# auduno/headtrackr

Hardware: AMD Instinct MI355X
Metric: frames/sec full-cascade detect at 320x240 (higher is better)
Workload: dtype u8; 1 GPU; C2: 256 x 320x240 RGBA frames per GPU, full BBF cascade detect (interval 5) incl. grouping + best face per frame on the host; frames_per_gpu=256, frames_total=256, width=320, height=240, batches_in_flight=3, parallelism=1 GPU

## Files before the change

### headtrackr_amd/csrc/ht_context.hip

```cpp
#include <sched.h>
#include <algorithm>
#include <cmath>
#include <cstddef>
#include <cstdlib>
#include <cstring>
#include <new>

#include "ht_internal.h"
#include "ht_hostpost.h"
#include "ht_geometry_plan.h"
#include "ht_cascade_plan.h"

static thread_local std::string g_create_err;

#include <dlfcn.h>
namespace {
struct Roctx {
    int (*push)(const char *) = nullptr;
    int (*pop)() = nullptr;
    Roctx() {
        void *h = dlopen("libroctx64.so", RTLD_NOW | RTLD_GLOBAL);
        if (!h) h = dlopen("libroctx64.so.4", RTLD_NOW | RTLD_GLOBAL);
        if (h) {
            push = reinterpret_cast<int (*)(const char *)>(dlsym(h, "roctxRangePushA"));
            pop = reinterpret_cast<int (*)()>(dlsym(h, "roctxRangePop"));
            if (!push || !pop) push = nullptr, pop = nullptr;
        }
    }
};
Roctx &roctx() {
    static Roctx r;
    return r;
}
}
HtRange::HtRange(const char *name) : on(roctx().push != nullptr) {
    if (on) roctx().push(name);
}
HtRange::~HtRange() {
    if (on) roctx().pop();
}

#include <atomic>
#include <mutex>
static std::mutex g_live_mu;
static std::vector<ht_ctx *> g_live;
struct HtOrphan {
    void *p;
    size_t bytes;
    int device;
    bool orphan;
};
static std::vector<HtOrphan> g_orphans;
static std::atomic<int> g_orphan_count{0};

static bool bound_by_live_context(const ht_ctx *except, int device, const void *p, size_t bytes) {
    const uint8_t *pb = static_cast<const uint8_t *>(p);
    for (const ht_ctx *o : g_live)
        if (o != except && o->device == device && o->d_frames && o->d_frames >= pb && o->d_frames < pb + bytes) return true;
    return false;
}

static void sweep_orphans(ht_ctx *c) {
    if (g_orphan_count.load(std::memory_order_relaxed) == 0) return;
    std::vector<HtOrphan> release;
    {
        std::lock_guard<std::mutex> lk(g_live_mu);
        for (size_t i = 0; i < g_orphans.size();) {
            if (!bound_by_live_context(nullptr, g_orphans[i].device, g_orphans[i].p, g_orphans[i].bytes)) {
                release.push_back(g_orphans[i]);
                g_orphans.erase(g_orphans.begin() + (long)i);
            } else {
                i++;
            }
        }
        g_orphan_count.store((int)g_orphans.size(), std::memory_order_relaxed);
    }
    for (auto &a : release) {
        (void)hipSetDevice(a.device);
        (void)hipDeviceSynchronize();
        (void)hipFree(a.p);
    }
    if (!release.empty() && c) (void)hipSetDevice(c->device);
}

static inline HtPostCfg post_cfg(const ht_ctx *c) { return HtPostCfg{c->interval, c->cascade.cw, c->cascade.ch}; }

static int ht_host_workers(const ht_ctx *c, int frames, uint32_t hits) {
    if (c->host_threads == 0) return 0;
    if (c->host_threads > 0) return c->host_threads;
    if (frames < 32 || hits < 256) return 0;
    static const int share = [] {
        cpu_set_t set;
        CPU_ZERO(&set);
        int cpus = sched_getaffinity(0, sizeof(set), &set) == 0 ? CPU_COUNT(&set) : (int)std::thread::hardware_concurrency();
        int ngpu = 1;
        if (hipGetDeviceCount(&ngpu) != hipSuccess || ngpu < 1) ngpu = 1;
        return std::max(0, std::min(7, cpus / (2 * ngpu) - 1));
    }();
    return share;
}


ht_status ht_fail(ht_ctx *ctx, ht_status st, const std::string &msg) {
    if (ctx)
        ctx->err = msg;
    else
        g_create_err = msg;
    return st;
}

HtProfScope::HtProfScope(ht_ctx *c, const char *name, hipStream_t on) : ctx(c), stream(on ? on : c->stream) {
    if (!ctx->profiling) return;
    for (size_t i = 0; i < ctx->timers.size(); i++)
        if (ctx->timers[i].name == name) idx = (int)i;
    if (idx < 0) {
        ctx->timers.emplace_back();
        ctx->timers.back().name = name;
        idx = (int)ctx->timers.size() - 1;
    }
    if (hipEventCreate(&a) != hipSuccess || hipEventCreate(&b) != hipSuccess) {
        idx = -1;
        return;
    }
    (void)hipEventRecord(a, stream);
}
HtProfScope::~HtProfScope() {
    if (idx < 0) return;
    (void)hipEventRecord(b, stream);
    ctx->timers[idx].pending.emplace_back(a, b);
    ctx->timers[idx].launches++;
}

extern "C" int32_t ht_abi_version(void) { return HT_ABI_VERSION; }

extern "C" const char *ht_last_error(const ht_ctx *ctx) { return ctx ? ctx->err.c_str() : g_create_err.c_str(); }

static bool apply_options(ht_ctx *c, const std::string &opts, std::string &why) {
    size_t pos = 0;
    while (pos < opts.size()) {
        size_t end = opts.find(',', pos);
        if (end == std::string::npos) end = opts.size();
        std::string kv = opts.substr(pos, end - pos);
        pos = end + 1;
        while (!kv.empty() && (kv.front() == ' ')) kv.erase(kv.begin());
        while (!kv.empty() && (kv.back() == ' ')) kv.pop_back();
        if (kv.empty()) continue;
        const size_t eq = kv.find('=');
        const std::string key = kv.substr(0, eq), val = eq == std::string::npos ? "1" : kv.substr(eq + 1);
        char *endp = nullptr;
        const long long v = std::strtoll(val.c_str(), &endp, 10);
        if (val.empty() || (endp && *endp)) {
            why = "option '" + key + "': value is not an integer";
            return false;
        }
        const int iv = (int)std::max<long long>(std::min<long long>(v, 1ll << 30), -(1ll << 30));
        if (key == "rs_rpt") { if (iv >= 1 && iv <= HT_RS_MAX_PASSES) c->rs_rpt = iv; }
        else if (key == "rs_tailtable") c->tail_table = iv < 0 ? 0 : (iv > 2 ? 2 : (int)iv), c->tail_table_forced = true;
        else if (key == "rs_tailcap") c->rs_tailcap = (uint64_t)std::max<long long>(v, 0), c->rs_tailcap_forced = true;
        else if (key == "rs_notail") c->rs_notail = iv != 0;
        else if (key == "rs_nofast") c->rs_nofast = iv != 0;
        else if (key == "rs_nosort") c->rs_nosort = iv != 0;
        else if (key == "rs_bands") c->rs_bands = iv != 0;
        else if (key == "rs_gennames") c->rs_gennames = iv != 0;
        else if (key == "rs_minwg") c->rs_min_wgs = std::max(1, iv);
        else if (key == "rs_k") c->dbg_rs_k = iv;
        else if (key == "rs_group") { if (iv >= 1 && iv <= 64) c->rs_group = iv, c->rs_group_forced = true; }
        else if (key == "early_scan") c->early_scan = iv != 0;
        else if (key == "force_exact") c->dbg_force_exact = iv;
        else if (key == "deep_bias") c->deep_bias = (uint32_t)std::max(0, iv);
        else if (key == "deep_v") c->dbg_deep_v = iv;
        else if (key == "cs_flags") c->cs_flags = iv != 0;
        else if (key == "cs_sync_ring") c->cs_sync_ring = iv != 0;
        else if (key == "cs_pairs_force") c->cs_pairs_force = iv != 0;
        else if (key == "cs_pairs_cluster") c->cs_pairs_cluster = iv != 0;
        else if (key == "fp_sparse") c->fp_sparse = iv != 0;
        else if (key == "deep_grid") c->deep_grid = std::max(1, iv);
        else if (key == "split") c->opt_split = std::max(1, iv);
        else if (key == "cs_fused_min") c->cs_fused_min_streams = std::max(1, iv);
        else if (key == "cs_fused_nt") c->cs_fused_nt = iv;
        else if (key == "cs_keep_hist") c->cs_keep_hist = iv != 0;
        else if (key == "cs_seq_fused") c->cs_seq_fused = iv != 0;
        else if (key == "cs_cluster") c->cs_cluster = iv != 0;
        else if (key == "cs_cluster_min_px") c->cs_cluster_min_px = (uint32_t)std::max(0, iv);
        else if (key == "cs_region") c->cs_region_cap = std::min(40960, std::max(0, iv));
        else if (key == "cs_barrier_budget") c->cs_barrier_budget = std::max(1ll, v);
        else if (key == "graph_max_frames") c->graph_max_frames = std::max(0, iv);
        else if (key == "host_threads") c->host_threads = std::min(64, std::max(0, iv));
        else if (key == "force_rccl") c->force_rccl = iv != 0;
        else if (key == "group_cap") c->grp_cap_opt = std::max(1, iv);
#ifdef HT_DEBUG_KNOBS
        else if (key == "stop_stage") c->dbg_stop_stage = iv;
        else if (key == "cs_iters") c->dbg_cs_iters = std::min(10, std::max(0, iv));
        else if (key == "rs_maxgen") c->rs_maxgen = iv;
#endif
        else {
            why = "unknown option '" + key + "'";
            return false;
        }
    }
    return true;
}

template <typename T>
static ht_status upload_table(ht_ctx *c, T *&dst, const std::vector<T> &src) {
    if (src.empty()) return HT_OK;
    HT_HIP(c, hipMalloc(&dst, src.size() * sizeof(T)));
    HT_HIP(c, hipMemcpy(dst, src.data(), src.size() * sizeof(T), hipMemcpyHostToDevice));
    return HT_OK;
}

extern "C" ht_status ht_create(const ht_config *cfg, const void *cascade_blob, size_t cascade_len, ht_ctx **out) {
    if (!cfg || !out || (cfg->struct_size != sizeof(ht_config) && cfg->struct_size != offsetof(ht_config, options)))
        return ht_fail(nullptr, HT_ERR_INVALID, "ht_create: bad config");
    *out = nullptr;
    if (cfg->interval < 1 || cfg->interval > 12) return ht_fail(nullptr, HT_ERR_INVALID, "ht_create: interval must be 1..12");
    int ndev = 0;
    if (hipGetDeviceCount(&ndev) != hipSuccess || ndev <= 0)
        return ht_fail(nullptr, HT_ERR_NO_DEVICE, "ht_create: no HIP device visible (this library has no CPU fallback)");
    if (cfg->device < 0 || cfg->device >= ndev) return ht_fail(nullptr, HT_ERR_INVALID, "ht_create: device ordinal out of range");
    hipDeviceProp_t prop;
    if (hipGetDeviceProperties(&prop, cfg->device) != hipSuccess) return ht_fail(nullptr, HT_ERR_HIP, "hipGetDeviceProperties failed");
    if (std::strncmp(prop.gcnArchName, "gfx950", 6) != 0)
        return ht_fail(nullptr, HT_ERR_NO_DEVICE, std::string("ht_create: device is ") + prop.gcnArchName + ", this build is gfx950-only");
    ht_ctx *c = new (std::nothrow) ht_ctx();
    if (!c) return ht_fail(nullptr, HT_ERR_NOMEM, "ht_create: out of host memory");
    c->device = cfg->device;
    c->num_cus = prop.multiProcessorCount > 0 ? prop.multiProcessorCount : 256;
    c->interval = cfg->interval;
    c->next = cfg->interval + 1;
    if (cfg->hit_capacity) c->hit_capacity = cfg->hit_capacity;
    c->queue_capacity_cfg = cfg->queue_capacity;
    std::string why;
    if (!ht_plan_cascade((const uint8_t *)cascade_blob, cascade_len, &c->cascade, &why)) {
        delete c;
        return ht_fail(nullptr, HT_ERR_INVALID, "ht_create: " + why);
    }
    ht_status st = HT_OK;
    auto bail = [&](ht_status s) {
        g_create_err = c->err;
        ht_destroy(c);
        return s;
    };
    if (hipSetDevice(c->device) != hipSuccess) {
        c->err = "hipSetDevice failed";
        return bail(HT_ERR_HIP);
    }
    if (cfg->stream) {
        c->stream = (hipStream_t)cfg->stream;
    } else {
        if (hipStreamCreateWithFlags(&c->stream, hipStreamNonBlocking) != hipSuccess) {
            c->err = "hipStreamCreate failed";
            return bail(HT_ERR_HIP);
        }
        c->own_stream = true;
    }
    {
        std::string opts = (cfg->struct_size >= offsetof(ht_config, options) + sizeof(const char *) && cfg->options) ? cfg->options : "";
#ifdef HT_DEBUG_KNOBS
        if (const char *e = std::getenv("HT_OPTIONS")) opts += std::string(opts.empty() ? "" : ",") + e;
#endif
        std::string why;
        if (!apply_options(c, opts, why)) {
            c->err = "ht_create: " + why;
            return bail(HT_ERR_INVALID);
        }
    }
    if (c->early_scan) {
        if (hipStreamCreateWithFlags(&c->aux_stream, hipStreamNonBlocking) != hipSuccess || hipEventCreateWithFlags(&c->ev_early_ready, hipEventDisableTiming) != hipSuccess ||
            hipEventCreateWithFlags(&c->ev_early_done, hipEventDisableTiming) != hipSuccess) {
            c->err = "hipStreamCreate (aux) failed";
            return bail(HT_ERR_HIP);
        }
    }
    c->builtin_cascade = ht_scan_is_builtin_cascade((const uint8_t *)cascade_blob, cascade_len) && c->interval >= 1;
    ht_plan_cascade_split(&c->cascade, c->builtin_cascade, c->opt_split);
    const HtCascadePlan &P = c->cascade;
    if ((st = upload_table(c, c->d_deep_feats, P.deep)) != HT_OK || (st = upload_table(c, c->d_stages, P.dev_stages)) != HT_OK ||
        (st = upload_table(c, c->d_tile_feats, P.tile)) != HT_OK || (st = upload_table(c, c->d_fp_feats, P.fp)) != HT_OK ||
        (st = upload_table(c, c->d_patch_feats, P.patch)) != HT_OK || (st = upload_table(c, c->d_packed_feats, P.packed)) != HT_OK)
        return bail(st);
    if (hipHostMalloc(reinterpret_cast<void **>(&c->h_pinned), sizeof(HtCounters) + (size_t)HT_PINNED_HITS * sizeof(ht_hit), hipHostMallocDefault) != hipSuccess ||
        hipMalloc(&c->d_stats, sizeof(unsigned long long) * 64 * HT_STAT_SHARDS) != hipSuccess ||
        hipMalloc(reinterpret_cast<void **>(&c->d_counters), sizeof(HtCounters) + (size_t)c->hit_capacity * sizeof(ht_hit)) != hipSuccess) {
        c->err = "hipMalloc(hits) failed";
        return bail(HT_ERR_NOMEM);
    }
    {
        std::lock_guard<std::mutex> lk(g_live_mu);
        g_live.push_back(c);
    }
    c->d_hits = reinterpret_cast<ht_hit *>(reinterpret_cast<uint8_t *>(c->d_counters) + sizeof(HtCounters));
    *out = c;
    return HT_OK;
}

static void destroy_graphs(ht_ctx *c);
static void free_geometry(ht_ctx *c) {
    destroy_graphs(c);
    if (c->d_levels) (void)hipFree(c->d_levels), c->d_levels = nullptr;
    if (c->d_arena) (void)hipFree(c->d_arena), c->d_arena = nullptr;
    if (c->d_scales) (void)hipFree(c->d_scales), c->d_scales = nullptr;
    if (c->d_queue) (void)hipFree(c->d_queue), c->d_queue = nullptr;
    for (auto p : c->d_gen_blocks)
        if (p) (void)hipFree(p);
    c->d_gen_blocks.clear();
    if (c->d_tile_recs) (void)hipFree(c->d_tile_recs), c->d_tile_recs = nullptr;
    if (c->d_tail_jobs) (void)hipFree(c->d_tail_jobs), c->d_tail_jobs = nullptr;
    if (c->d_tail_prefix) (void)hipFree(c->d_tail_prefix), c->d_tail_prefix = nullptr;
    if (c->d_tail_taps) (void)hipFree(c->d_tail_taps), c->d_tail_taps = nullptr;
    if (c->d_tail_taps_fast) (void)hipFree(c->d_tail_taps_fast), c->d_tail_taps_fast = nullptr;
    if (c->d_tail_tapref) (void)hipFree(c->d_tail_tapref), c->d_tail_tapref = nullptr;
    c->plan.tail_first_gen = 0;
    c->plan.gens.clear();
    c->plan.gen_blocks.clear();
    c->plan.scales.clear();
}

extern "C" void ht_destroy(ht_ctx *c) {
    if (!c) return;
    std::vector<HtOrphan> release;
    {
        std::lock_guard<std::mutex> lk(g_live_mu);
        g_live.erase(std::remove(g_live.begin(), g_live.end(), c), g_live.end());
        for (auto &a : c->user_allocs) {
            if (bound_by_live_context(c, c->device, a.first, a.second)) g_orphans.push_back(HtOrphan{a.first, a.second, c->device, true});
            else release.push_back(HtOrphan{a.first, a.second, c->device, false});
        }
        c->user_allocs.clear();
        for (size_t i = 0; i < g_orphans.size();) {
            if (!bound_by_live_context(nullptr, g_orphans[i].device, g_orphans[i].p, g_orphans[i].bytes)) {
                release.push_back(g_orphans[i]);
                g_orphans.erase(g_orphans.begin() + (long)i);
            } else {
                i++;
            }
        }
        g_orphan_count.store((int)g_orphans.size(), std::memory_order_relaxed);
    }
    (void)hipSetDevice(c->device);
    if (c->stream) (void)hipStreamSynchronize(c->stream);
    if (c->aux_stream) (void)hipStreamSynchronize(c->aux_stream), (void)hipStreamDestroy(c->aux_stream);
    if (c->ev_early_ready) (void)hipEventDestroy(c->ev_early_ready);
    if (c->ev_early_done) (void)hipEventDestroy(c->ev_early_done);
    free_geometry(c);
    if (c->d_tile_feats) (void)hipFree(c->d_tile_feats);
    if (c->d_deep_feats) (void)hipFree(c->d_deep_feats);
    if (c->d_patch_feats) (void)hipFree(c->d_patch_feats);
    if (c->d_packed_feats) (void)hipFree(c->d_packed_feats);
    if (c->d_fp_feats) (void)hipFree(c->d_fp_feats);
    if (c->d_stages) (void)hipFree(c->d_stages);
    if (c->d_frames_own) (void)hipFree(c->d_frames_own);
    if (c->d_frames_back) (void)hipFree(c->d_frames_back);
    if (c->ev_copy_done) (void)hipEventDestroy(c->ev_copy_done);
    if (c->ev_front_free) (void)hipEventDestroy(c->ev_front_free);
    if (c->copy_stream) (void)hipStreamDestroy(c->copy_stream);
    if (c->d_counters) (void)hipFree(c->d_counters);
    if (c->d_stats) (void)hipFree(c->d_stats);
    if (c->h_pinned) (void)hipHostFree(c->h_pinned);
    if (c->d_scratch) (void)hipFree(c->d_scratch);
    if (c->h_wb_pinned) (void)hipHostFree(c->h_wb_pinned);
    ht_camshift_free(c);
    ht_backproject_free(c);
    ht_ingest_free(c);
    ht_cs_pairs_free(c);
    ht_cs_best_free(c);
    ht_group_free(c);
    if (c->d_gather) (void)hipFree(c->d_gather);
    for (auto &a : release) {
        if (a.orphan) {
            (void)hipSetDevice(a.device);
            (void)hipDeviceSynchronize();
        }
        (void)hipFree(a.p);
    }
    (void)hipSetDevice(c->device);
    for (auto &t : c->timers)
        for (auto &p : t.pending) (void)hipEventDestroy(p.first), (void)hipEventDestroy(p.second);
    if (c->own_stream && c->stream) (void)hipStreamDestroy(c->stream);
    delete c;
}


static ht_status set_geometry_impl(ht_ctx *c, int32_t width, int32_t height, int32_t max_batch, const int32_t *level_dims, int n, int upto) {
    c->W = width;
    c->H = height;
    c->max_batch = max_batch;
    c->nlevels = n;
    c->upto = upto;

    HtPlanInputs in;
    in.interval = c->interval, in.next = c->next, in.cw = c->cascade.cw, in.ch = c->cascade.ch;
    in.rs_rpt = c->rs_rpt, in.rs_nofast = c->rs_nofast, in.rs_nosort = c->rs_nosort, in.rs_notail = c->rs_notail;
    in.rs_tailcap = c->rs_tailcap, in.rs_tailcap_forced = c->rs_tailcap_forced;
    in.tail_table = c->tail_table, in.tail_table_forced = c->tail_table_forced;
    in.early_scan = c->early_scan, in.aux_stream = c->aux_stream != nullptr;
    in.queue_capacity_cfg = c->queue_capacity_cfg;
    HtGeometryPlan &P = c->plan;
    std::string why;
    ht_status st = ht_plan_geometry(in, width, height, max_batch, level_dims, n, upto, &P, &why);
    if (st != HT_OK) return ht_fail(c, st, why);

    c->d_gen_blocks.assign(P.gens.size(), nullptr);
    for (size_t g = 1; g < P.gens.size(); g++)
        if ((st = upload_table(c, c->d_gen_blocks[g], P.gen_tiles[g])) != HT_OK) return st;
    HT_HIP(c, hipMalloc(&c->d_levels, sizeof(HtDevLevel) * HT_MAX_LEVELS));
    HT_HIP(c, hipMemcpy(c->d_levels, P.levels, sizeof(HtDevLevel) * n, hipMemcpyHostToDevice));
    if (hipMalloc(&c->d_arena, P.arena_stride * (uint64_t)max_batch) != hipSuccess)
        return ht_fail(c, HT_ERR_NOMEM, "ht_set_geometry: hipMalloc(pyramid arena) failed");
    HT_HIP(c, hipMemset(c->d_arena, 0, P.arena_stride * (uint64_t)max_batch));
    if ((st = upload_table(c, c->d_tail_jobs, P.tail_jobs)) != HT_OK || (st = upload_table(c, c->d_tail_prefix, P.tail_prefix)) != HT_OK ||
        (st = upload_table(c, c->d_tail_taps, P.tail_taps)) != HT_OK || (st = upload_table(c, c->d_tail_taps_fast, P.tail_taps_fast)) != HT_OK ||
        (st = upload_table(c, c->d_tail_tapref, P.tail_tapref)) != HT_OK || (st = upload_table(c, c->d_tile_recs, P.tile_recs)) != HT_OK ||
        (st = upload_table(c, c->d_scales, P.scales)) != HT_OK)
        return st;
    if (hipMalloc(&c->d_queue, (size_t)P.queue_capacity * sizeof(HtQueueEntry) + HT_DEEP_CTR_BYTES) != hipSuccess)
        return ht_fail(c, HT_ERR_NOMEM, "ht_set_geometry: hipMalloc(survivor queue) failed");
    return HT_OK;
}

extern "C" ht_status ht_set_geometry(ht_ctx *c, int32_t width, int32_t height, int32_t max_batch, const int32_t *level_dims,
                                     int32_t nlevels_in) {
    if (!c) return HT_ERR_INVALID;
    if (width <= 0 || height <= 0 || width > 16384 || height > 16384 || max_batch <= 0)
        return ht_fail(c, HT_ERR_INVALID, "ht_set_geometry: width/height must be 1..16384 and max_batch > 0");
    HT_HIP(c, hipSetDevice(c->device));
    const int upto = (int)std::floor(std::log((double)std::min(c->cascade.cw, c->cascade.ch)) / std::log(ht_scale_of(c->interval)));
    const int n = upto + c->next * 2;
    if (n > HT_MAX_LEVELS) return ht_fail(c, HT_ERR_INVALID, "ht_set_geometry: too many pyramid levels");
    if (level_dims && nlevels_in != n) return ht_fail(c, HT_ERR_INVALID, "ht_set_geometry: level_dims has the wrong number of levels");
    if (level_dims)
        for (int i = 0; i < n; i++) {
            const int lw = level_dims[2 * i], lh = level_dims[2 * i + 1];
            if (lw < 0 || lh < 0 || lw > width || lh > height || (i == 0 && (lw != width || lh != height)))
                return ht_fail(c, HT_ERR_INVALID, "ht_set_geometry: bad level_dims");
        }
    if (c->W == width && c->H == height && c->max_batch >= max_batch && c->nlevels == n && !level_dims) return HT_OK;
    HT_HIP(c, hipStreamSynchronize(c->stream));
    if (c->copy_stream) HT_HIP(c, hipStreamSynchronize(c->copy_stream));
    free_geometry(c);
    c->nframes = c->enq_nframes = 0;
    c->wb_collected_n = -1;
    c->back_n = 0;
    c->d_frames = nullptr;
    c->enqueued = false;
    const ht_status st = set_geometry_impl(c, width, height, max_batch, level_dims, n, upto);
    if (st != HT_OK) {
        (void)hipGetLastError();
        free_geometry(c);
        c->W = c->H = c->max_batch = c->nlevels = c->upto = 0;
    }
    return st;
}

extern "C" int32_t ht_num_levels(const ht_ctx *c) { return c ? c->nlevels : 0; }
extern "C" uint64_t ht_windows_per_frame(const ht_ctx *c) { return c ? c->plan.windows_per_frame : 0; }
extern "C" uint64_t ht_pyramid_bytes_per_frame(const ht_ctx *c) { return c ? c->plan.pyr_bytes : 0; }

extern "C" ht_status ht_plane(const ht_ctx *c, int32_t level, int32_t slot, ht_plane_info *out) {
    if (!c || !out || level < 0 || level >= c->nlevels || slot < 0 || slot > 3) return HT_ERR_INVALID;
    const HtDevLevel &L = c->plan.levels[level];
    out->width = L.w;
    out->height = L.h;
    out->stride = L.stride;
    out->present = L.off[slot] != 0xffffffffu;
    out->offset = out->present ? L.off[slot] : 0;
    return HT_OK;
}


extern "C" ht_status ht_upload_frames(ht_ctx *c, const uint8_t *host_rgba, int32_t n, size_t frame_stride) {
    if (!c) return HT_ERR_INVALID;
    HtRange range("ht_upload_frames");
    if (c->W == 0) return ht_fail(c, HT_ERR_STATE, "ht_upload_frames: call ht_set_geometry first");
    const size_t fbytes = (size_t)c->W * c->H * 4;
    if (!host_rgba || n <= 0 || n > c->max_batch || frame_stride < fbytes)
        return ht_fail(c, HT_ERR_INVALID, "ht_upload_frames: bad frame count or stride");
    HT_HIP(c, hipSetDevice(c->device));
    const size_t need = fbytes * (size_t)n;
    const ht_status st = ht_frames_own_reserve(c, need, "ht_upload_frames");
    if (st != HT_OK) return st;
    if (frame_stride == fbytes) {
        HT_HIP(c, hipMemcpyAsync(c->d_frames_own, host_rgba, need, hipMemcpyHostToDevice, c->stream));
    } else {
        HT_HIP(c, hipMemcpy2DAsync(c->d_frames_own, fbytes, host_rgba, frame_stride, fbytes, (size_t)n, hipMemcpyHostToDevice, c->stream));
    }
    ht_frames_bind_own(c, n);
    return HT_OK;
}

ht_status ht_frames_own_reserve(ht_ctx *c, size_t need, const char *fn) {
    if (c->d_frames_own_bytes >= need) return HT_OK;
    HT_HIP(c, hipStreamSynchronize(c->stream));
    if (c->d_frames == c->d_frames_own) c->d_frames = nullptr, c->nframes = 0;
    if (c->d_frames_own) (void)hipFree(c->d_frames_own);
    c->d_frames_own = nullptr;
    c->d_frames_own_bytes = 0;
    if (hipMalloc(&c->d_frames_own, need) != hipSuccess) return (void)hipGetLastError(), ht_fail(c, HT_ERR_NOMEM, std::string(fn) + ": hipMalloc failed");
    c->d_frames_own_bytes = need;
    return HT_OK;
}
void ht_frames_bind_own(ht_ctx *c, int n) {
    c->d_frames = c->d_frames_own;
    c->frame_stride = (size_t)c->W * c->H * 4;
    c->nframes = n;
    sweep_orphans(c);
}

extern "C" ht_status ht_upload_frames_async(ht_ctx *c, const uint8_t *host_rgba, int32_t n, size_t frame_stride) {
    if (!c) return HT_ERR_INVALID;
    if (c->W == 0) return ht_fail(c, HT_ERR_STATE, "ht_upload_frames_async: call ht_set_geometry first");
    const size_t fbytes = (size_t)c->W * c->H * 4;
    if (!host_rgba || n <= 0 || n > c->max_batch || frame_stride < fbytes)
        return ht_fail(c, HT_ERR_INVALID, "ht_upload_frames_async: bad frame count or stride");
    HT_HIP(c, hipSetDevice(c->device));
    if (!c->copy_stream) {
        HT_HIP(c, hipStreamCreateWithFlags(&c->copy_stream, hipStreamNonBlocking));
        HT_HIP(c, hipEventCreateWithFlags(&c->ev_copy_done, hipEventDisableTiming));
        HT_HIP(c, hipEventCreateWithFlags(&c->ev_front_free, hipEventDisableTiming));
    }
    const size_t need = fbytes * (size_t)n;
    if (c->d_frames_back_bytes < need) {
        HT_HIP(c, hipStreamSynchronize(c->copy_stream));
        if (c->d_frames_back) (void)hipFree(c->d_frames_back);
        c->d_frames_back = nullptr;
        c->d_frames_back_bytes = 0;
        if (hipMalloc(&c->d_frames_back, need) != hipSuccess) return ht_fail(c, HT_ERR_NOMEM, "ht_upload_frames_async: hipMalloc failed");
        c->d_frames_back_bytes = need;
    }
    HT_HIP(c, hipStreamWaitEvent(c->copy_stream, c->ev_front_free, 0));
    if (frame_stride == fbytes) {
        HT_HIP(c, hipMemcpyAsync(c->d_frames_back, host_rgba, need, hipMemcpyHostToDevice, c->copy_stream));
    } else {
        HT_HIP(c, hipMemcpy2DAsync(c->d_frames_back, fbytes, host_rgba, frame_stride, fbytes, (size_t)n, hipMemcpyHostToDevice, c->copy_stream));
    }
    HT_HIP(c, hipEventRecord(c->ev_copy_done, c->copy_stream));
    c->back_n = n;
    return HT_OK;
}

extern "C" ht_status ht_swap_frames(ht_ctx *c) {
    if (!c) return HT_ERR_INVALID;
    if (c->back_n <= 0) return ht_fail(c, HT_ERR_STATE, "ht_swap_frames: no ht_upload_frames_async pending");
    HT_HIP(c, hipSetDevice(c->device));
    HT_HIP(c, hipEventRecord(c->ev_front_free, c->stream));
    HT_HIP(c, hipStreamWaitEvent(c->stream, c->ev_copy_done, 0));
    std::swap(c->d_frames_own, c->d_frames_back);
    std::swap(c->d_frames_own_bytes, c->d_frames_back_bytes);
    c->d_frames = c->d_frames_own;
    c->frame_stride = (size_t)c->W * c->H * 4;
    c->nframes = c->back_n;
    c->back_n = 0;
    sweep_orphans(c);
    return HT_OK;
}

extern "C" ht_status ht_bind_frames_device(ht_ctx *c, const void *dev_rgba, int32_t n, size_t frame_stride) {
    if (!c) return HT_ERR_INVALID;
    if (c->W == 0) return ht_fail(c, HT_ERR_STATE, "ht_bind_frames_device: call ht_set_geometry first");
    if (!dev_rgba || n <= 0 || n > c->max_batch || frame_stride < (size_t)c->W * c->H * 4 || (frame_stride & 3) ||
        ((uintptr_t)dev_rgba & 3))
        return ht_fail(c, HT_ERR_INVALID, "ht_bind_frames_device: bad pointer, frame count or stride (4-byte alignment required)");
    c->d_frames = (const uint8_t *)dev_rgba;
    c->frame_stride = frame_stride;
    c->nframes = n;
    sweep_orphans(c);
    return HT_OK;
}

extern "C" int32_t ht_frames_bound(const ht_ctx *c) { return c ? c->nframes : 0; }
extern "C" int32_t ht_frames_enqueued(const ht_ctx *c) { return (c && c->enqueued) ? c->enq_nframes : 0; }

extern "C" ht_status ht_host_alloc(size_t bytes, void **out) {
    if (!out || bytes == 0) return HT_ERR_INVALID;
    *out = nullptr;
    if (hipHostMalloc(out, bytes, hipHostMallocDefault) != hipSuccess) {
        (void)hipGetLastError();
        return ht_fail(nullptr, HT_ERR_NOMEM, "ht_host_alloc: hipHostMalloc failed");
    }
    return HT_OK;
}
extern "C" void ht_host_free(void *p) {
    if (p) (void)hipHostFree(p);
}
extern "C" ht_status ht_device_alloc(ht_ctx *c, size_t bytes, void **out) {
    if (!c || !out || bytes == 0) return HT_ERR_INVALID;
    *out = nullptr;
    HT_HIP(c, hipSetDevice(c->device));
    if (hipMalloc(out, bytes) != hipSuccess) {
        (void)hipGetLastError();
        return ht_fail(c, HT_ERR_NOMEM, "ht_device_alloc: hipMalloc failed");
    }
    c->user_allocs.emplace_back(*out, bytes);
    return HT_OK;
}
extern "C" ht_status ht_device_free(ht_ctx *c, void *p) {
    if (!c) return HT_ERR_INVALID;
    if (!p) return HT_OK;
    HT_HIP(c, hipSetDevice(c->device));
    HT_HIP(c, hipStreamSynchronize(c->stream));
    auto it = std::find_if(c->user_allocs.begin(), c->user_allocs.end(), [p](const std::pair<void *, size_t> &a) { return a.first == p; });
    if (it == c->user_allocs.end()) return ht_fail(c, HT_ERR_INVALID, "ht_device_free: not a live ht_device_alloc buffer of this context");
    const uint8_t *pb = static_cast<const uint8_t *>(p);
    {
        std::lock_guard<std::mutex> lk(g_live_mu);
        if (bound_by_live_context(c, c->device, pb, it->second))
            return ht_fail(c, HT_ERR_STATE, "ht_device_free: another live context still has frames bound inside this buffer (rebind or destroy it first)");
    }
    if (c->d_frames && c->d_frames >= pb && c->d_frames < pb + it->second) {
        c->d_frames = nullptr, c->nframes = 0;
        destroy_graphs(c);
    }
    c->user_allocs.erase(it);
    HT_HIP(c, hipFree(p));
    sweep_orphans(c);
    return HT_OK;
}
extern "C" ht_status ht_device_upload(ht_ctx *c, void *dst_dev, const void *src_host, size_t bytes) {
    if (!c || !dst_dev || !src_host) return HT_ERR_INVALID;
    if (bytes == 0) return HT_OK;
    HT_HIP(c, hipSetDevice(c->device));
    HT_HIP(c, hipMemcpyAsync(dst_dev, src_host, bytes, hipMemcpyHostToDevice, c->stream));
    HT_HIP(c, hipStreamSynchronize(c->stream));
    return HT_OK;
}

extern "C" ht_status ht_device_download(ht_ctx *c, void *dst_host, const void *src_dev, size_t bytes) {
    if (!c || !dst_host || !src_dev) return HT_ERR_INVALID;
    if (bytes == 0) return HT_OK;
    HT_HIP(c, hipSetDevice(c->device));
    HT_HIP(c, hipMemcpyAsync(dst_host, src_dev, bytes, hipMemcpyDeviceToHost, c->stream));
    HT_HIP(c, hipStreamSynchronize(c->stream));
    return HT_OK;
}


static ht_status wb_scratch(ht_ctx *c) {
    const size_t region = sizeof(unsigned long long) * 4 * (size_t)std::max(c->max_batch, 1), need = 2 * region;
    if (c->d_scratch_bytes < need) {
        HT_HIP(c, hipStreamSynchronize(c->stream));
        destroy_graphs(c);
        if (c->d_scratch) (void)hipFree(c->d_scratch);
        c->d_scratch = nullptr;
        c->d_scratch_bytes = 0;
        if (hipMalloc(&c->d_scratch, need) != hipSuccess) return ht_fail(c, HT_ERR_NOMEM, "whitebalance scratch: hipMalloc failed");
        c->d_scratch_bytes = need;
    }
    if (c->h_wb_pinned_bytes < region) {
        HT_HIP(c, hipStreamSynchronize(c->stream));
        if (c->h_wb_pinned) (void)hipHostFree(c->h_wb_pinned);
        c->h_wb_pinned = nullptr;
        c->h_wb_pinned_bytes = 0;
        if (hipHostMalloc(reinterpret_cast<void **>(&c->h_wb_pinned), region, hipHostMallocDefault) != hipSuccess)
            return ht_fail(c, HT_ERR_NOMEM, "whitebalance staging: hipHostMalloc failed");
        c->h_wb_pinned_bytes = region;
    }
    return HT_OK;
}
static unsigned long long *wb_standalone_region(ht_ctx *c) {
    return reinterpret_cast<unsigned long long *>(c->d_scratch) + 4 * (size_t)std::max(c->max_batch, 1);
}

static ht_status detect_enqueue_body(ht_ctx *c, uint32_t flags) {
    HT_HIP(c, hipMemsetAsync(c->d_counters, 0, sizeof(HtCounters), c->stream));
    c->early_launched = false;
    if (flags & HT_SCAN_STATS) HT_HIP(c, hipMemsetAsync(c->d_stats, 0, sizeof(unsigned long long) * 64 * HT_STAT_SHARDS, c->stream));
    ht_status st;
    c->wb_fused = false;
    const bool wb = (flags & HT_DETECT_WHITEBALANCE) != 0;
    if (wb) {
        HT_HIP(c, hipMemsetAsync(c->d_scratch, 0, sizeof(unsigned long long) * 4 * (size_t)c->nframes, c->stream));
        c->wb_fused = (c->W & 3) == 0;
    }
    st = ht_launch_pyramid(c, flags);
    c->wb_fused = false;
    if (st != HT_OK) return st;
    if (wb && (c->W & 3) != 0 && (st = ht_launch_whitebalance(c, c->d_scratch, false)) != HT_OK) return st;
    return ht_launch_scan(c, flags);
}

static void destroy_graphs(ht_ctx *c) {
    for (auto &g : c->graphs) {
        if (g.exec) (void)hipGraphExecDestroy(g.exec);
        if (g.graph) (void)hipGraphDestroy(g.graph);
    }
    c->graphs.clear();
}

extern "C" uint64_t ht_graph_launches(const ht_ctx *c) { return c ? c->graph_launches : 0; }

extern "C" ht_status ht_detect_enqueue(ht_ctx *c, uint32_t flags) {
    if (!c) return HT_ERR_INVALID;
    HtRange range("ht_detect_enqueue");
    if (!c->d_frames || c->nframes <= 0) return ht_fail(c, HT_ERR_STATE, "ht_detect_enqueue: no frames bound");
    HT_HIP(c, hipSetDevice(c->device));
    ht_status st;
    if ((flags & HT_DETECT_WHITEBALANCE) && (st = wb_scratch(c)) != HT_OK) return st;
    const bool graph_ok = c->graph_max_frames > 0 && c->nframes <= c->graph_max_frames && c->own_stream && !c->profiling && !c->early_scan &&
                          !(flags & HT_SCAN_STATS);
    bool done = false;
    if (graph_ok) {
        HtDetectGraph *g = nullptr;
        for (auto &e : c->graphs)
            if (e.frames == c->d_frames && e.frame_stride == c->frame_stride && e.nframes == c->nframes && e.flags == flags) g = &e;
        if (!g) {
            if (c->graphs.size() >= 8) {
                HtDetectGraph &old = c->graphs.front();
                if (old.exec) (void)hipGraphExecDestroy(old.exec);
                if (old.graph) (void)hipGraphDestroy(old.graph);
                c->graphs.erase(c->graphs.begin());
            }
            c->graphs.emplace_back();
            g = &c->graphs.back();
            g->frames = c->d_frames, g->frame_stride = c->frame_stride, g->nframes = c->nframes, g->flags = flags;
        }
        if (!g->exec && g->seen == 1) {
            ht_capture_mark(c, true);
            if (hipStreamBeginCapture(c->stream, hipStreamCaptureModeThreadLocal) == hipSuccess) {
                st = detect_enqueue_body(c, flags);
                hipGraph_t graph = nullptr;
                const hipError_t e = hipStreamEndCapture(c->stream, &graph);
                ht_capture_mark(c, false);
                if (st == HT_OK && e == hipSuccess && graph && hipGraphInstantiate(&g->exec, graph, nullptr, nullptr, 0) == hipSuccess) {
                    g->graph = graph;
                } else {
                    if (graph) (void)hipGraphDestroy(graph);
                    g->exec = nullptr;
                    g->seen = 1 << 30;
                    (void)hipGetLastError();
                }
            } else {
                ht_capture_mark(c, false);
                (void)hipGetLastError();
                g->seen = 1 << 30;
            }
        }
        if (g->exec) {
            HT_HIP(c, hipGraphLaunch(g->exec, c->stream));
            c->graph_launches++;
            c->early_launched = false;
            done = true;
        } else if (g->seen < (1 << 30)) {
            g->seen++;
        }
    }
    if (!done && (st = detect_enqueue_body(c, flags)) != HT_OK) return st;
    c->stats_enqueued = (flags & HT_SCAN_STATS) != 0;
    c->wb_enqueued = (flags & HT_DETECT_WHITEBALANCE) != 0;
    c->enqueued = true;
    c->grp_enqueued = false;
    c->enq_nframes = c->nframes;
    return HT_OK;
}

ht_status ht_detect_mark_collected(ht_ctx *c, bool wb_snap) {
    c->enqueued = false;
    if (wb_snap) {
        c->h_wb_sums.assign(c->h_wb_pinned, c->h_wb_pinned + 4 * (size_t)c->enq_nframes);
        c->wb_collected_n = c->enq_nframes;
    } else {
        c->wb_collected_n = -1;
    }
    std::memset(c->h_stage_in, 0, sizeof(c->h_stage_in));
    if (c->stats_enqueued) {
        std::vector<unsigned long long> sh((size_t)64 * HT_STAT_SHARDS);
        HT_HIP(c, hipMemcpy(sh.data(), c->d_stats, sh.size() * sizeof(unsigned long long), hipMemcpyDeviceToHost));
        for (int r = 0; r < HT_STAT_SHARDS; r++)
            for (int j = 0; j < 64; j++) c->h_stage_in[j] += sh[(size_t)r * 64 + j];
    }
    return HT_OK;
}

static inline bool hit_less(const ht_hit &a, const ht_hit &b) {
    if (a.frame != b.frame) return a.frame < b.frame;
    if (a.scale != b.scale) return a.scale < b.scale;
    if (a.q != b.q) return a.q < b.q;
    if (a.y != b.y) return a.y < b.y;
    return a.x < b.x;
}

extern "C" ht_status ht_detect_collect(ht_ctx *c, ht_hit *hits, uint32_t cap, uint32_t *counts, uint32_t *total) {
    if (!c) return HT_ERR_INVALID;
    HtRange range("ht_detect_collect");
    if (!c->enqueued) return ht_fail(c, HT_ERR_STATE, "ht_detect_collect: nothing enqueued");
    HT_HIP(c, hipSetDevice(c->device));
    uint32_t spec = std::max<uint32_t>(256u, 64u * (uint32_t)std::max(c->enq_nframes, 1));
    if (c->spec_hint) spec = std::min(spec, std::max<uint32_t>(256u, c->spec_hint + c->spec_hint / 2 + 64u));
    spec = std::min<uint32_t>(spec, std::min<uint32_t>(HT_PINNED_HITS, c->hit_capacity));
    HT_HIP(c, hipMemcpyAsync(c->h_pinned, c->d_counters, sizeof(HtCounters) + (size_t)spec * sizeof(ht_hit), hipMemcpyDeviceToHost, c->stream));
    const bool wb_snap = c->wb_enqueued && c->h_wb_pinned;
    if (wb_snap)
        HT_HIP(c, hipMemcpyAsync(c->h_wb_pinned, c->d_scratch, sizeof(unsigned long long) * 4 * (size_t)c->enq_nframes, hipMemcpyDeviceToHost, c->stream));
    HT_HIP(c, hipStreamSynchronize(c->stream));
    std::memcpy(&c->h_counters, c->h_pinned, sizeof(HtCounters));
    c->grp_enqueued = false;
    const ht_status cst = ht_detect_mark_collected(c, wb_snap);
    if (cst != HT_OK) return cst;
    const uint32_t found = c->h_counters.nhits;
    c->spec_hint = found;
    if (total) *total = found;
    const uint32_t nfr = (uint32_t)c->enq_nframes;
    if (counts) std::memset(counts, 0, sizeof(uint32_t) * (size_t)nfr);
    if (found > c->hit_capacity)
        return ht_fail(c, HT_ERR_CAPACITY, "ht_detect_collect: more raw hits than ht_config.hit_capacity; results incomplete");
    std::vector<ht_hit> &tmp = c->h_raw_hits;
    tmp.resize(found);
    if (found) {
        const uint32_t have = std::min(found, spec);
        std::memcpy(tmp.data(), c->h_pinned + sizeof(HtCounters), (size_t)have * sizeof(ht_hit));
        if (found > have)
            HT_HIP(c, hipMemcpy(tmp.data() + have, c->d_hits + have, (size_t)(found - have) * sizeof(ht_hit), hipMemcpyDeviceToHost));
    }
    if (c->requeue_flags >= 0) {
        const uint32_t fl = (uint32_t)c->requeue_flags;
        c->requeue_flags = -1;
        ht_status rq = ht_detect_enqueue(c, fl);
        if (rq != HT_OK) return rq;
    }
    const uint32_t ncopy = std::min(found, cap);
    ht_hit *dst = hits;
    if (found && (!hits || cap < found)) {
        c->h_ordered_hits.resize(found);
        dst = c->h_ordered_hits.data();
    }
    bool bucketed = found > 0 && nfr > 0;
    if (bucketed) {
        bucketed = ht_post_bucket_by_frame(tmp.data(), found, nfr, dst, c->h_frame_start, counts);
        if (bucketed) {
            const uint32_t *se = c->h_frame_start.data();
            if (c->collect_best_follows) {
                c->h_sort_deferred = true;
            } else {
                auto sort_frames = [&](int f0, int f1) {
                    for (int f = f0; f < f1; f++) ht_post_sort_frame(dst, f ? se[f - 1] : 0u, se[f]);
                };
                const int nw = ht_host_workers(c, (int)nfr, found);
                if (nw > 0) HtPool::get().run((int)nfr, 16, nw, sort_frames);
                else sort_frames(0, (int)nfr);
            }
        }
    }
    if (found && !bucketed) {
        std::sort(tmp.begin(), tmp.end(), hit_less);
        if (counts) {
            std::memset(counts, 0, sizeof(uint32_t) * (size_t)nfr);
            for (uint32_t i = 0; i < found; i++)
                if (tmp[i].frame < nfr) counts[tmp[i].frame]++;
        }
        std::memcpy(dst, tmp.data(), (size_t)found * sizeof(ht_hit));
    }
    if (found && dst != hits && hits && ncopy) std::memcpy(hits, dst, (size_t)ncopy * sizeof(ht_hit));
    if (found > cap) return ht_fail(c, HT_ERR_CAPACITY, "ht_detect_collect: caller buffer too small for all hits");
    return HT_OK;
}

extern "C" ht_status ht_detect_batch(ht_ctx *c, const uint8_t *host_rgba, int32_t n, int32_t width, int32_t height, size_t frame_stride,
                                     uint32_t flags, ht_hit *hits, uint32_t cap, uint32_t *counts, uint32_t *total) {
    if (!c) return HT_ERR_INVALID;
    ht_status st;
    if (c->W != width || c->H != height || c->max_batch < n)
        if ((st = ht_set_geometry(c, width, height, n, nullptr, 0)) != HT_OK) return st;
    if ((st = ht_upload_frames(c, host_rgba, n, frame_stride)) != HT_OK) return st;
    if ((st = ht_detect_enqueue(c, flags)) != HT_OK) return st;
    return ht_detect_collect(c, hits, cap, counts, total);
}

extern "C" ht_status ht_pyramid_readback(ht_ctx *c, int32_t frame, int32_t level, int32_t slot, uint8_t *out, size_t cap) {
    if (!c || !out) return HT_ERR_INVALID;
    if (frame < 0 || frame >= c->max_batch || level < 0 || level >= c->nlevels || slot < 0 || slot > 3)
        return ht_fail(c, HT_ERR_INVALID, "ht_pyramid_readback: index out of range");
    const HtDevLevel &L = c->plan.levels[level];
    if (L.off[slot] == 0xffffffffu) return ht_fail(c, HT_ERR_INVALID, "ht_pyramid_readback: plane does not exist");
    if (cap < (size_t)L.w * L.h) return ht_fail(c, HT_ERR_CAPACITY, "ht_pyramid_readback: buffer too small");
    if (L.w == 0 || L.h == 0) return HT_OK;
    HT_HIP(c, hipSetDevice(c->device));
    HT_HIP(c, hipStreamSynchronize(c->stream));
    HT_HIP(c, hipMemcpy2D(out, L.w, c->d_arena + (uint64_t)frame * c->plan.arena_stride + L.off[slot], L.stride, L.w, L.h, hipMemcpyDeviceToHost));
    return HT_OK;
}

extern "C" ht_status ht_stage_counts(ht_ctx *c, uint64_t *counts, int32_t n) {
    if (!c || !counts || n < (int32_t)c->cascade.nstages + 1) return HT_ERR_INVALID;
    for (uint32_t j = 0; j <= c->cascade.nstages; j++) counts[j] = c->h_stage_in[j];
    for (int32_t j = (int32_t)c->cascade.nstages + 1; j < std::min<int32_t>(n, 64); j++) counts[j] = c->h_stage_in[j];
    return HT_OK;
}

extern "C" ht_status ht_grayscale_batch(ht_ctx *c, uint8_t *host_rgba, int32_t n, int32_t width, int32_t height, size_t frame_stride) {
    if (!c || !host_rgba || n <= 0 || width <= 0 || height <= 0 || frame_stride < (size_t)width * height * 4) return HT_ERR_INVALID;
    HT_HIP(c, hipSetDevice(c->device));
    const size_t fbytes = (size_t)width * height * 4;
    uint8_t *d = nullptr;
    if (hipMalloc(&d, fbytes * n) != hipSuccess) return ht_fail(c, HT_ERR_NOMEM, "ht_grayscale_batch: hipMalloc failed");
    ht_status st = HT_OK;
    hipError_t e = hipMemcpy2DAsync(d, fbytes, host_rgba, frame_stride, fbytes, n, hipMemcpyHostToDevice, c->stream);
    if (e == hipSuccess) {
        const int W0 = c->W, H0 = c->H;
        c->W = width, c->H = height;
        st = ht_launch_gray_inplace(c, d, n, fbytes);
        c->W = W0, c->H = H0;
    }
    if (e == hipSuccess && st == HT_OK) e = hipMemcpy2DAsync(host_rgba, frame_stride, d, fbytes, fbytes, n, hipMemcpyDeviceToHost, c->stream);
    if (e == hipSuccess) e = hipStreamSynchronize(c->stream);
    (void)hipFree(d);
    if (e != hipSuccess) return ht_fail(c, HT_ERR_HIP, std::string("ht_grayscale_batch: ") + hipGetErrorString(e));
    return st;
}

static void wb_values(const ht_ctx *c, const unsigned long long *sums, double *out, int32_t n) {
    const double imagesize = (double)c->W * (double)c->H;
    for (int i = 0; i < n; i++) {
        const double avgr = (double)sums[4 * i] / imagesize, avgg = (double)sums[4 * i + 1] / imagesize, avgb = (double)sums[4 * i + 2] / imagesize;
        out[i] = (avgr + avgg + avgb) / 3;
    }
}

extern "C" ht_status ht_whitebalance_batch(ht_ctx *c, double *out, int32_t n) {
    if (!c || !out) return HT_ERR_INVALID;
    if (!c->d_frames || n <= 0 || n > c->nframes) return ht_fail(c, HT_ERR_STATE, "ht_whitebalance_batch: no frames bound");
    HT_HIP(c, hipSetDevice(c->device));
    ht_status st = wb_scratch(c);
    if (st != HT_OK) return st;
    unsigned long long *d_sums = wb_standalone_region(c);
    if ((st = ht_launch_whitebalance(c, reinterpret_cast<double *>(d_sums), true)) != HT_OK) return st;
    std::vector<unsigned long long> sums((size_t)n * 4);
    HT_HIP(c, hipMemcpyAsync(sums.data(), d_sums, sizeof(unsigned long long) * 4 * (size_t)n, hipMemcpyDeviceToHost, c->stream));
    HT_HIP(c, hipStreamSynchronize(c->stream));
    wb_values(c, sums.data(), out, n);
    return HT_OK;
}

extern "C" ht_status ht_detect_whitebalance(ht_ctx *c, double *out, int32_t n) {
    if (!c || !out) return HT_ERR_INVALID;
    if (c->wb_collected_n < 0)
        return ht_fail(c, HT_ERR_STATE, "ht_detect_whitebalance: the batch collected last was not enqueued with HT_DETECT_WHITEBALANCE (call after ht_detect_collect)");
    if (n <= 0 || n > c->wb_collected_n) return ht_fail(c, HT_ERR_INVALID, "ht_detect_whitebalance: n exceeds the collected batch");
    wb_values(c, c->h_wb_sums.data(), out, n);
    return HT_OK;
}


extern "C" ht_status ht_hits_to_rects(const ht_ctx *c, const ht_hit *hits, uint32_t n, ht_rect *out) {
    if (!c || (n && (!hits || !out))) return HT_ERR_INVALID;
    const HtPostCfg cfg = post_cfg(c);
    double sx[HT_MAX_LEVELS];
    ht_post_level_scales(cfg, sx);
    return ht_post_hits_to_rects(cfg, sx, hits, n, out);
}

extern "C" ht_status ht_group_rects(const ht_rect *seq, uint32_t n, int32_t min_neighbors, ht_rect *out, uint32_t *nout) {
    return ht_post_group_rects(seq, n, min_neighbors, out, nout);
}

extern "C" ht_status ht_best_faces(const ht_ctx *c, const ht_hit *hits, const uint32_t *counts, int32_t nframes, int32_t min_neighbors,
                                   ht_rect *best) {
    if (!c || !counts || !best || nframes < 0) return HT_ERR_INVALID;
    const HtPostCfg cfg = post_cfg(c);
    double sx[HT_MAX_LEVELS];
    ht_post_level_scales(cfg, sx);
    size_t k = 0;
    for (int f = 0; f < nframes; f++) {
        const ht_status st = ht_post_best_face(cfg, sx, hits ? hits + k : nullptr, counts[f], min_neighbors, &best[f]);
        if (st != HT_OK) return st;
        k += counts[f];
    }
    return HT_OK;
}

extern "C" ht_status ht_detect_collect_best(ht_ctx *c, int32_t min_neighbors, ht_rect *best, uint32_t *total_hits) {
    if (!c || !best) return HT_ERR_INVALID;
    HtRange range("ht_detect_collect_best");
    if (!c->enqueued) return ht_fail(c, HT_ERR_STATE, "ht_detect_collect_best: nothing enqueued");
    const int nfr = c->enq_nframes;
    if (c->h_collect_hits.size() < (size_t)c->hit_capacity) c->h_collect_hits.resize(c->hit_capacity);
    c->h_collect_counts.resize((size_t)std::max(nfr, 1));
    uint32_t total = 0;
    c->collect_best_follows = true;
    c->h_sort_deferred = false;
    ht_status st = ht_detect_collect(c, c->h_collect_hits.data(), c->hit_capacity, c->h_collect_counts.data(), &total);
    c->collect_best_follows = false;
    if (total_hits) *total_hits = total;
    if (st != HT_OK) return st;
    if (!c->h_sort_deferred) return ht_best_faces(c, c->h_collect_hits.data(), c->h_collect_counts.data(), nfr, min_neighbors, best);
    return ht_post_frames(post_cfg(c), c->h_collect_hits.data(), c->h_frame_start.data(), nfr, min_neighbors, ht_host_workers(c, nfr, total), best);
}

extern "C" ht_status ht_detect_collect_best_requeue(ht_ctx *c, int32_t min_neighbors, ht_rect *best, uint32_t *total_hits, uint32_t next_flags) {
    if (!c || !best) return HT_ERR_INVALID;
    if (!c->enqueued) return ht_fail(c, HT_ERR_STATE, "ht_detect_collect_best_requeue: nothing enqueued");
    c->requeue_flags = (int64_t)next_flags;
    const ht_status st = ht_detect_collect_best(c, min_neighbors, best, total_hits);
    c->requeue_flags = -1;
    return st;
}


extern "C" ht_status ht_profile(ht_ctx *c, int32_t on) {
    if (!c) return HT_ERR_INVALID;
    c->profiling = on != 0;
    return HT_OK;
}

extern "C" ht_status ht_kernel_times(ht_ctx *c, ht_kernel_time *out, int32_t *n, int32_t reset) {
    if (!c || !n) return HT_ERR_INVALID;
    HT_HIP(c, hipSetDevice(c->device));
    HT_HIP(c, hipStreamSynchronize(c->stream));
    for (auto &t : c->timers) {
        for (auto &p : t.pending) {
            float ms = 0;
            if (hipEventElapsedTime(&ms, p.first, p.second) == hipSuccess) t.ms += ms;
            (void)hipEventDestroy(p.first);
            (void)hipEventDestroy(p.second);
        }
        t.pending.clear();
    }
    const int cap = *n;
    int k = 0;
    for (auto &t : c->timers) {
        if (out && k < cap) {
            std::memset(&out[k], 0, sizeof(ht_kernel_time));
            std::strncpy(out[k].name, t.name.c_str(), sizeof(out[k].name) - 1);
            out[k].ms = t.ms;
            out[k].launches = t.launches;
        }
        k++;
    }
    static const char *const form_names[2] = {"cs_fused_launches_1024", "cs_fused_launches_512"};
    for (int f = 0; f < 2; f++) {
        if (!c->cs_fused_launches[f]) continue;
        if (out && k < cap) {
            std::memset(&out[k], 0, sizeof(ht_kernel_time));
            std::strncpy(out[k].name, form_names[f], sizeof(out[k].name) - 1);
            out[k].launches = c->cs_fused_launches[f];
        }
        k++;
    }
    if (c->grp_over_cap_frames) {
        if (out && k < cap) {
            std::memset(&out[k], 0, sizeof(ht_kernel_time));
            std::strncpy(out[k].name, "grp_over_cap_frames", sizeof(out[k].name) - 1);
            out[k].launches = c->grp_over_cap_frames;
        }
        k++;
    }
    *n = k;
    if (reset) c->timers.clear(), c->cs_fused_launches[0] = c->cs_fused_launches[1] = 0, c->grp_over_cap_frames = 0;
    return HT_OK;
}

extern "C" void *ht_stream(const ht_ctx *c) { return c ? (void *)c->stream : nullptr; }

extern "C" ht_status ht_synchronize(ht_ctx *c) {
    if (!c) return HT_ERR_INVALID;
    HT_HIP(c, hipSetDevice(c->device));
    HT_HIP(c, hipStreamSynchronize(c->stream));
    return HT_OK;
}
```

### headtrackr_amd/csrc/ht_geometry_plan.h

```cpp
#pragma once

#include <algorithm>
#include <cmath>
#include <cstring>
#include <string>
#include <vector>

#include "ht_hostpost.h"
#include "ht_plan_types.h"

static inline uint64_t align_up(uint64_t v, uint64_t a) { return (v + a - 1) / a * a; }

static HtTap ht_host_tap(int i, double r, int s, int origin) {
    double f = ((double)i + 0.5) * r;
    f = f + (-0.5);
    f = f < 0.0 ? 0.0 : f;
    const double fmax = (double)(s - 1);
    f = f > fmax ? fmax : f;
    const double af = std::floor(f);
    HtTap tp;
    tp.a = origin + (int)af;
    tp.b = origin + std::min((int)af + 1, s - 1);
    tp.t = f - af;
    tp.u = 1.0 - tp.t;
    return tp;
}

static ht_status ht_plan_levels(const HtPlanInputs &in, int width, int height, const int32_t *level_dims, int n, HtGeometryPlan *p, std::string *why) {
    const int next = in.next;
    uint64_t off = 0;
    p->pyr_bytes = 0;
    for (int i = 0; i < n; i++) {
        HtDevLevel &L = p->levels[i];
        if (level_dims) {
            L.w = level_dims[2 * i];
            L.h = level_dims[2 * i + 1];
        } else if (i == 0) {
            L.w = width;
            L.h = height;
        } else if (i <= in.interval) {
            L.w = (int)std::floor((double)width / ht_scale_pow(in.interval, i));
            L.h = (int)std::floor((double)height / ht_scale_pow(in.interval, i));
        } else {
            L.w = p->levels[i - next].w / 2;
            L.h = p->levels[i - next].h / 2;
        }
        L.stride = (int)align_up((uint64_t)L.w, 4);
        for (int s = 0; s < 4; s++) {
            if (s == 0 || i >= 2 * next) {
                if (off > 0xfffffff0ull) return *why = "ht_set_geometry: frame too large", HT_ERR_INVALID;
                L.off[s] = (uint32_t)off;
                off = align_up(off + (uint64_t)L.stride * L.h, 256);
                p->pyr_bytes += (uint64_t)L.w * L.h;
            } else {
                L.off[s] = 0xffffffffu;
            }
        }
    }
    p->arena_stride = align_up(off + 256, 256);
    return HT_OK;
}

static void ht_plan_jobs(const HtPlanInputs &in, int n, HtGeometryPlan *p, std::vector<int> &gen) {
    const int next = in.next;
    gen.assign(n, 0);
    int ngen = 1;
    for (int i = 1; i < n; i++) {
        gen[i] = (i <= in.interval) ? 1 : gen[i - next] + 1;
        ngen = std::max(ngen, gen[i] + 1);
    }
    p->gens.assign(ngen, {});
    auto add_job = [&](int g, int src, int dst, int slot, int sx, int sy, int sw, int sh, int dw, int dh) {
        const HtDevLevel &S = p->levels[src], &D = p->levels[dst];
        if (D.w <= 0 || D.h <= 0) return;
        HtResampleJob j;
        std::memset(&j, 0, sizeof(j));
        j.src_off = S.off[0];
        j.dst_off = D.off[slot];
        j.src_stride = S.stride;
        j.dst_stride = D.stride;
        j.sx = sx, j.sy = sy, j.sw = sw, j.sh = sh;
        j.dw = dw, j.dh = dh;
        j.cw = D.w, j.ch = D.h;
        if (sw <= 0 || sh <= 0 || dw <= 0 || dh <= 0) {
            j.dw = j.dh = 0;
            j.sw = j.sh = 1;
            j.rx = j.ry = 1;
        } else {
            j.rx = (double)sw / (double)dw;
            j.ry = (double)sh / (double)dh;
        }
        p->gens[g].push_back(j);
    };
    for (int i = 1; i < n; i++) {
        const HtDevLevel &D = p->levels[i];
        if (i <= in.interval) {
            add_job(gen[i], 0, i, 0, 0, 0, p->levels[0].w, p->levels[0].h, D.w, D.h);
        } else {
            const HtDevLevel &S = p->levels[i - next];
            add_job(gen[i], i - next, i, 0, 0, 0, S.w, S.h, D.w, D.h);
            if (i >= 2 * next) {
                add_job(gen[i], i - next, i, 1, 1, 0, S.w - 1, S.h, D.w - 2, D.h);
                add_job(gen[i], i - next, i, 2, 0, 1, S.w, S.h - 1, D.w, D.h - 2);
                add_job(gen[i], i - next, i, 3, 1, 1, S.w - 1, S.h - 1, D.w - 2, D.h - 2);
            }
        }
    }
}

static std::vector<HtResampleJob> ht_plan_gen_tiles(const HtPlanInputs &in, const std::vector<HtResampleJob> &jobs) {
    std::vector<HtResampleJob> tiles;
    for (auto &j : jobs) {
        int npmax = 1;
        for (int t = 2; t <= std::min(in.rs_rpt, HT_RS_MAX_PASSES); t++)
            if ((int)std::ceil(16.0 * t * j.ry) + 3 <= HT_RS_SRC_ROWS) npmax = t;
        const int passes = (j.ch + 15) / 16, nby = (passes + npmax - 1) / npmax, nbx = (j.cw + 63) / 64;
        int pass0 = 0;
        for (int y = 0; y < nby; y++) {
            const int np = passes / nby + (y < passes % nby ? 1 : 0);
            for (int x = 0; x < nbx; x++) {
                HtResampleJob t = j;
                t.bx = (uint16_t)x, t.pass0 = (uint16_t)pass0, t.np = (uint16_t)np;
                t.pad = in.rs_nofast ? 2 : (uint16_t)((j.dw > 0 && j.sw == 2 * j.dw && j.sh == 2 * j.dh) ? 1 : 0);
                const int X0 = 64 * x, Y0 = 16 * pass0, ncols = std::min(64, j.dw - X0), nrows = std::min(16 * np, j.dh - Y0);
                if (ncols > 0 && nrows > 0) {
                    t.ex_xa = ht_host_tap(X0, j.rx, j.sw, j.sx).a & ~15;
                    t.ex_ya = ht_host_tap(Y0, j.ry, j.sh, j.sy).a;
                    t.ex_sw16 = (ht_host_tap(X0 + ncols - 1, j.rx, j.sw, j.sx).b - t.ex_xa) / 16 + 1;
                    t.ex_sh = ht_host_tap(Y0 + nrows - 1, j.ry, j.sh, j.sy).b - t.ex_ya + 1;
                    bool fit = t.ex_sw16 * 16 <= 160;
                    for (int w = 0; w < 4; w++) {
                        const int r0 = std::min(4 * np * w, nrows - 1), r1 = std::min(4 * np * (w + 1) - 1, nrows - 1);
                        const int bya = ht_host_tap(Y0 + r0, j.ry, j.sh, j.sy).a - t.ex_ya;
                        const int bsh = ht_host_tap(Y0 + r1, j.ry, j.sh, j.sy).b - (t.ex_ya + bya) + 1;
                        if (bya < 0 || bya > 255 || bsh < 1 || bsh > HT_RSB_ROWS) fit = false;
                        t.band_ya4 |= (uint32_t)(bya & 0xff) << (8 * w), t.band_sh4 |= (uint32_t)(bsh & 0xff) << (8 * w);
                    }
                    if (fit) t.pad |= 4;
                }
                tiles.push_back(t);
            }
            pass0 += np;
        }
    }
    if (!in.rs_nosort)
        std::stable_sort(tiles.begin(), tiles.end(), [](const HtResampleJob &a, const HtResampleJob &b) {
            if (a.src_off != b.src_off) return a.src_off < b.src_off;
            const int ya = (int)(16.0 * a.pass0 * a.ry), yb = (int)(16.0 * b.pass0 * b.ry);
            if (ya / 32 != yb / 32) return ya < yb;
            return a.bx < b.bx;
        });
    return tiles;
}

static void ht_plan_tail(const HtPlanInputs &in, int max_batch, HtGeometryPlan *p) {
    const int ngen = (int)p->gens.size();
    constexpr int HT_SMALL_BATCH = 48;
    const uint64_t tail_cap = in.rs_tailcap_forced ? in.rs_tailcap : (max_batch <= HT_SMALL_BATCH ? 4000u : in.rs_tailcap);
    p->tail_table = in.tail_table_forced ? in.tail_table : ((max_batch <= 128 && max_batch > HT_SMALL_BATCH) ? 1 : 0);
    p->tail_first_gen = 0;
    if (in.rs_notail) return;
    int g0 = ngen;
    uint64_t px = 0;
    for (int g = ngen - 1; g >= 1; g--) {
        uint64_t gp = 0;
        for (auto &j : p->gens[g]) gp += (uint64_t)j.cw * j.ch;
        if (p->gens[g].size() > (size_t)HT_TAIL_MAX_JOBS || px + gp > tail_cap) break;
        px += gp;
        g0 = g;
    }
    if (!(ngen - g0 >= 2 && ngen - g0 <= HT_TAIL_MAX_GENS)) return;
    std::vector<HtResampleJob> &tj = p->tail_jobs;
    std::vector<uint32_t> &pref = p->tail_prefix;
    HtTailGens &T = p->tail;
    std::memset(&T, 0, sizeof(T));
    T.ngen = ngen - g0;
    for (int g = g0; g < ngen; g++) {
        T.job_begin[g - g0] = (int32_t)tj.size();
        uint32_t groups = 0;
        for (auto &j : p->gens[g]) {
            tj.push_back(j);
            pref.push_back(groups);
            groups += (uint32_t)((j.cw + 3) / 4) * (uint32_t)j.ch;
        }
        T.groups[g - g0] = groups;
    }
    T.job_begin[T.ngen] = (int32_t)tj.size();
    if (tj.empty()) return;
    std::vector<HtTap> &taps = p->tail_taps;
    std::vector<HtTapFast> &fast = p->tail_taps_fast;
    std::vector<HtTailTapRef> &refs = p->tail_tapref;
    const bool nofast = in.rs_nofast;
    size_t jidx = 0;
    for (auto &j : tj) {
        for (int g = 0; g <= T.ngen; g++)
            if ((size_t)T.job_begin[g] == jidx) T.tap_begin[g] = (uint32_t)taps.size();
        jidx++;
        HtTailTapRef r;
        r.col = (uint32_t)taps.size();
        const int ncol = std::max(j.dw, 1), nrow = std::max(j.dh, 1);
        for (int i = 0; i < ncol + 3; i++) taps.push_back(ht_host_tap(std::min(i, ncol - 1), j.rx, j.sw, j.sx));
        r.row = (uint32_t)taps.size();
        for (int i = 0; i < nrow; i++) taps.push_back(ht_host_tap(i, j.ry, j.sh, j.sy));
        r.mode = nofast ? 2u : ((j.dw > 0 && j.sw == 2 * j.dw && j.sh == 2 * j.dh) ? 1u : 0u);
        r.pad = 0;
        refs.push_back(r);
    }
    T.tap_begin[T.ngen] = (uint32_t)taps.size();
    fast.resize(taps.size());
    for (size_t i = 0; i < taps.size(); i++) fast[i].a = taps[i].a, fast[i].tf = (float)taps[i].t;
    p->tail_first_gen = g0;
}

static ht_status ht_plan_scan_tiles(const HtPlanInputs &in, int upto, HtGeometryPlan *p, std::string *why) {
    constexpr int TXH = HT_SCAN_TXH, TYH = HT_SCAN_TYH;
    p->scales.clear();
    p->windows_per_frame = 0;
    uint32_t tiles = 0;
    for (int i = 0; i < upto; i++) {
        HtScanScale S;
        std::memset(&S, 0, sizeof(S));
        S.l0 = i;
        S.l1 = i + in.next;
        S.l2 = i + 2 * in.next;
        S.qw = p->levels[S.l2].w - (int)(in.cw / 4);
        S.qh = p->levels[S.l2].h - (int)(in.ch / 4);
        if (S.qw <= 0 || S.qh <= 0) continue;
        S.ntx = (2 * S.qw + TXH - 1) / TXH;
        S.tw2 = (2 * S.qw + S.ntx - 1) / S.ntx;
        S.tw2 = (S.tw2 + 7) & ~7;
        S.nty = (2 * S.qh + TYH - 1) / TYH;
        S.th2 = (2 * S.qh + S.nty - 1) / S.nty;
        S.th2 += S.th2 & 1;
        S.ntx = (2 * S.qw + S.tw2 - 1) / S.tw2;
        S.nty = (2 * S.qh + S.th2 - 1) / S.th2;
        S.tile_begin = tiles;
        S.div_magic = ((1u << 20) + (uint32_t)S.tw2 - 1) / (uint32_t)S.tw2;
        if (p->windows_per_frame + 4ull * S.qw * S.qh > 0xffffffffull) return *why = "frame too large", HT_ERR_INVALID;
        S.win_begin = (uint32_t)p->windows_per_frame;
        tiles += (uint32_t)(S.ntx * S.nty);
        p->windows_per_frame += 4ull * (uint64_t)S.qw * (uint64_t)S.qh;
        p->scales.push_back(S);
    }
    p->tiles_per_frame = tiles;
    std::vector<HtTileRec> &recs = p->tile_recs;
    for (const HtScanScale &S : p->scales) {
        const HtDevLevel &A = p->levels[S.l0], &B = p->levels[S.l1], &Cq = p->levels[S.l2];
        if (A.stride > 0xffff || A.h > 0xffff) return *why = "frame too large", HT_ERR_INVALID;
        for (int y = 0; y < S.nty; y++)
            for (int x = 0; x < S.ntx; x++) {
                HtTileRec r;
                std::memset(&r, 0, sizeof(r));
                const int X0 = x * S.tw2, Y0 = y * S.th2;
                r.off0 = A.off[0], r.off1 = B.off[0];
                for (int q = 0; q < 4; q++) r.off2[q] = Cq.off[q];
                r.sh0 = (uint32_t)A.stride | (uint32_t)A.h << 16;
                r.sh1 = (uint32_t)B.stride | (uint32_t)B.h << 16;
                r.sh2 = (uint32_t)Cq.stride | (uint32_t)Cq.h << 16;
                r.origin = (uint32_t)X0 | (uint32_t)Y0 << 16;
                r.size = (uint32_t)std::min(S.tw2, 2 * S.qw - X0) | (uint32_t)std::min(S.th2, 2 * S.qh - Y0) << 16;
                r.tw2_l0 = (uint32_t)S.tw2 | (uint32_t)S.l0 << 16;
                r.div_magic = S.div_magic;
                {
                    const uint32_t th = r.size >> 16, d = 4u * th;
                    r.strip_magic = ((1u << 24) + d - 1u) / d;
                    for (uint32_t n = 0; n < (uint32_t)(S.tw2 / 2) * th; n++)
                        if (((n * r.strip_magic) >> 24) != n / d) return *why = "tile plan: strip_magic is not exact", HT_ERR_INVALID;
                }
                recs.push_back(r);
            }
    }
    return HT_OK;
}

static void ht_plan_early_split(const HtPlanInputs &in, const std::vector<int> &gen, HtGeometryPlan *p) {
    const int ngen = (int)p->gens.size();
    p->early_gen = 0;
    p->early_tiles = 0;
    if (in.early_scan && in.aux_stream && ngen > 3 && (p->tail_first_gen == 0 || p->tail_first_gen > 2)) {
        uint32_t tiles = 0;
        for (auto &S : p->scales) {
            if (gen[S.l2] > 2) break;
            tiles += (uint32_t)(S.ntx * S.nty);
        }
        if (tiles > 0 && tiles < p->tiles_per_frame) p->early_gen = 2, p->early_tiles = tiles;
    }
}

static ht_status ht_plan_geometry(const HtPlanInputs &in, int width, int height, int max_batch, const int32_t *level_dims, int n, int upto,
                                  HtGeometryPlan *plan, std::string *why) {
    *plan = HtGeometryPlan();
    ht_status st = ht_plan_levels(in, width, height, level_dims, n, plan, why);
    if (st != HT_OK) return st;
    std::vector<int> gen;
    ht_plan_jobs(in, n, plan, gen);
    const int ngen = (int)plan->gens.size();
    plan->gen_tiles.assign(ngen, {});
    plan->gen_blocks.assign(ngen, 0);
    for (int g = 1; g < ngen; g++) {
        plan->gen_tiles[g] = ht_plan_gen_tiles(in, plan->gens[g]);
        plan->gen_blocks[g] = (uint32_t)plan->gen_tiles[g].size();
    }
    ht_plan_tail(in, max_batch, plan);
    if ((st = ht_plan_scan_tiles(in, upto, plan, why)) != HT_OK) return st;
    ht_plan_early_split(in, gen, plan);
    uint64_t qc = in.queue_capacity_cfg ? in.queue_capacity_cfg : std::max<uint64_t>(1u << 16, plan->windows_per_frame * (uint64_t)max_batch / 8);
    qc = std::min<uint64_t>(qc, 1ull << 28);
    plan->queue_capacity = (uint32_t)qc;
    return HT_OK;
}
```

### headtrackr_amd/csrc/ht_internal.h

```cpp
#pragma once

#include <hip/hip_runtime.h>
#include <stdint.h>

#include <atomic>
#include <string>
#include <vector>

#include "headtrackr_hip.h"

#include "ht_cascade_types.h"

#include "ht_plan_types.h"

constexpr int HT_TAIL_LDS_TAPS = 4096;

struct HtBlockRef {
    uint16_t item;
    uint16_t bx, by;
    uint16_t pad;
};

struct alignas(16) HtQueueEntry {
    uint32_t frame;
    uint16_t x, y;
    uint8_t scale, q;
    uint16_t stage;
    uint32_t o0, o1, o2;
    uint16_t s0, s1, s2;
    uint16_t pad;
};
static_assert(sizeof(HtQueueEntry) == 32, "HtQueueEntry");

#define HT_DEEP_CTRS 16
#define HT_DEEP_CTR_BYTES (HT_DEEP_CTRS * 256)
#define HT_PINNED_HITS 8192
#define HT_STAT_SHARDS 256

struct HtCounters {
    uint32_t nhits;
    uint32_t nqueue;
    uint32_t queue_inline;
    uint32_t pad;
};

#include "ht_cs_schedule.h"

struct HtDetectGraph {
    const uint8_t *frames = nullptr;
    size_t frame_stride = 0;
    int nframes = 0;
    uint32_t flags = 0;
    int seen = 0;
    hipGraph_t graph = nullptr;
    hipGraphExec_t exec = nullptr;
};

struct HtKernelTimer {
    std::string name;
    double ms = 0;
    uint32_t launches = 0;
    std::vector<std::pair<hipEvent_t, hipEvent_t>> pending;
};

struct ht_ctx {
    int device = 0;
    hipStream_t stream = nullptr;
    bool own_stream = false;
    hipStream_t aux_stream = nullptr;
    hipEvent_t ev_early_ready = nullptr, ev_early_done = nullptr;
    bool early_scan = false;
    bool early_launched = false;
    std::string err;

    int interval = 5, next = 6;
    HtCascadePlan cascade;
    HtTileFeature *d_tile_feats = nullptr;
    HtDeepFeature *d_deep_feats = nullptr;
    HtPatchFeature *d_patch_feats = nullptr;
    HtPackedFeature *d_packed_feats = nullptr;
    HtPackedFeature *d_fp_feats = nullptr;
    bool fp_sparse = true;
    bool builtin_cascade = false;
    uint32_t deep_bias = 1;
    int dbg_stop_stage = -1, dbg_force_exact = 0, dbg_deep_v = 4, deep_grid = 192;
    HtDevStage *d_stages = nullptr;
    int opt_split = 0;

    int W = 0, H = 0, max_batch = 0, nlevels = 0, upto = 0;
    HtGeometryPlan plan;
    HtDevLevel *d_levels = nullptr;
    uint8_t *d_arena = nullptr;
    std::vector<HtResampleJob *> d_gen_blocks;
    HtTileRec *d_tile_recs = nullptr;
    HtScanScale *d_scales = nullptr;
    HtResampleJob *d_tail_jobs = nullptr;
    uint32_t *d_tail_prefix = nullptr;
    HtTap *d_tail_taps = nullptr;
    HtTapFast *d_tail_taps_fast = nullptr;
    HtTailTapRef *d_tail_tapref = nullptr;
    bool deep_attr_set = false;
    int tail_table = 1;
    bool tail_table_forced = false;
    bool rs_nofast = false, rs_nosort = false, rs_notail = false, rs_gennames = false;
    uint64_t rs_tailcap = 32768;
    bool rs_tailcap_forced = false;
    int rs_maxgen = 1 << 30;
    bool force_rccl = false;
    int host_threads = -1;
    int rs_min_wgs = 1536;
    int dbg_rs_k = 0;
    int rs_group = 8;
    bool rs_group_forced = false;
    int rs_rpt = 4;
    bool rs_bands = true;

    uint8_t *d_frames_own = nullptr;
    size_t d_frames_own_bytes = 0;
    uint8_t *d_frames_back = nullptr;
    size_t d_frames_back_bytes = 0;
    int back_n = 0;
    hipStream_t copy_stream = nullptr;
    hipEvent_t ev_copy_done = nullptr, ev_front_free = nullptr;
    const uint8_t *d_frames = nullptr;
    size_t frame_stride = 0;
    int nframes = 0;
    std::atomic<bool> capturing{false};
    int graph_max_frames = 256;
    std::vector<HtDetectGraph> graphs;
    uint64_t graph_launches = 0;
    int64_t requeue_flags = -1;
    int enq_nframes = 0;

    uint32_t hit_capacity = 1u << 20, queue_capacity_cfg = 0;
    ht_hit *d_hits = nullptr;
    HtQueueEntry *d_queue = nullptr;
    HtCounters *d_counters = nullptr;
    uint32_t spec_hint = 0;
    HtCounters h_counters;
    uint8_t *h_pinned = nullptr;
    unsigned long long *d_stats = nullptr;
    unsigned long long h_stage_in[64] = {0};
    std::vector<ht_hit> h_collect_hits;
    std::vector<uint32_t> h_collect_counts;
    std::vector<ht_hit> h_raw_hits;
    std::vector<ht_hit> h_ordered_hits;
    std::vector<uint32_t> h_frame_start;
    bool stats_enqueued = false;
    bool enqueued = false;
    bool collect_best_follows = false;
    bool h_sort_deferred = false;

    double *d_scratch = nullptr;
    size_t d_scratch_bytes = 0;
    bool wb_fused = false;
    bool wb_enqueued = false;
    unsigned long long *h_wb_pinned = nullptr;
    size_t h_wb_pinned_bytes = 0;
    std::vector<unsigned long long> h_wb_sums;
    int wb_collected_n = -1;

    int cs_streams = 0;
    HtCsState *d_cs = nullptr;
    uint32_t *d_cs_hist = nullptr;
    ht_cs_trackobj *d_cs_out = nullptr;
    double *d_cs_lut = nullptr, *d_cs_parts = nullptr;
    bool cs_cluster = true;
    uint32_t cs_cluster_min_px = 10000;
    ht_cs_trackobj *d_cs_seq_out = nullptr;
    size_t cs_seq_cap = 0;
    int cs_seq_pending_n = 0, cs_seq_pending_calls = 0, cs_seq_pending_all = 0;
    static constexpr int HT_CS_RING = 4;
    struct HtCsSlot {
        ht_cs_trackobj *h_out = nullptr;
        hipEvent_t ev = nullptr;
        int n = 0;
        uint32_t *h_flag = nullptr;
        uint32_t seq = 0;
    };
    ht_cs_rect *h_cs_rects = nullptr;
    int h_cs_rects_cap = 0;
    hipEvent_t ev_cs_rects = nullptr;
    uint32_t cs_flag_seq = 0;
    bool cs_flags = true;
    bool cs_sync_ring = true;
    HtCsSlot cs_ring[HT_CS_RING];
    int cs_ring_head = 0, cs_ring_count = 0, cs_ring_streams = 0;
    uint32_t *h_cs_err_direct = nullptr;
    uint32_t *d_cs_err = nullptr;
    uint32_t *h_cs_err = nullptr;
    long long cs_barrier_budget = 1ll << 28;
    int num_cus = 256;
    uint32_t cs_fused_launches[2] = {0, 0};
    int cs_fused_nt = 0;
    int cs_fused_min_streams = 192;
    bool cs_seq_attr_set = false;
    bool cs_seq_fused = true;
    int dbg_cs_iters = 10;
    bool cs_keep_hist = false;
    bool cs_attr_set = false;
    int cs_region_cap = 40960;
    int cs_last_first = 0, cs_last_n = 0, cs_last_chunks = 0;
    const uint32_t *cs_last_hist = nullptr;

    uint32_t *d_bp_hist = nullptr;
    double *d_bp_lut_w = nullptr;
    uint32_t *d_bp_lut_px = nullptr;
    uint8_t *d_bp_out = nullptr;
    size_t bp_hist_cap = 0, bp_lut_w_cap = 0, bp_lut_px_cap = 0, bp_out_cap = 0;

    static constexpr int HT_CSP_STAGE = 4;
    int32_t *d_csp_tab = nullptr;
    size_t csp_tab_cap = 0;
    int32_t *h_csp_tab[HT_CSP_STAGE] = {nullptr, nullptr, nullptr, nullptr};
    hipEvent_t ev_csp_tab[HT_CSP_STAGE] = {nullptr, nullptr, nullptr, nullptr};
    size_t h_csp_tab_cap = 0;
    int csp_stage_next = 0;
    uint32_t *d_csp_hist = nullptr;
    size_t csp_hist_cap = 0;
    bool csp_attr_set = false;
    bool cs_pairs_force = false;
    bool cs_pairs_cluster = false;
    std::vector<int32_t> cs_pair_slot;
    int cs_pair_chunks = 0;

    int32_t *d_csb_res = nullptr, *h_csb_res = nullptr;
    size_t csb_cap = 0;
    hipEvent_t ev_csb = nullptr;
    int csb_n = 0;
    const void *csb_states = nullptr;

    uint8_t *d_ingest_src = nullptr;
    size_t ingest_src_cap = 0;
    static constexpr int HT_DL_STAGE = 4;
    uint8_t *d_dl_tab = nullptr, *h_dl_tab[HT_DL_STAGE] = {};
    hipEvent_t ev_dl_tab[HT_DL_STAGE] = {};
    size_t dl_tab_cap = 0;
    int dl_stage_next = 0;

    std::vector<std::pair<void *, size_t>> user_allocs;

    int grp_cap_opt = 1 << 30;
    ht_hit *d_grp_hits2 = nullptr;
    ht_rect *d_grp_rects = nullptr;
    uint8_t *d_grp_out = nullptr, *h_grp_out = nullptr;
    size_t grp_out_cap = 0, h_grp_out_cap = 0;
    uint32_t *d_grp_cursor = nullptr;
    size_t grp_cursor_cap = 0;
    double *d_grp_konst = nullptr;
    ht_hit *d_grp_in = nullptr;
    size_t grp_in_cap = 0;
    bool grp_enqueued = false;
    bool grp_valid = false;
    int grp_nframes = 0;
    int32_t grp_min_neighbors = 1, grp_frame_base = 0;
    std::vector<uint32_t> h_grp_ngrouped, h_grp_start, h_grp_status;
    std::vector<std::vector<ht_rect>> h_grp_over;
    uint32_t grp_over_cap_frames = 0;

    void *d_gather = nullptr;
    size_t d_gather_bytes = 0;

    bool profiling = false;
    std::vector<HtKernelTimer> timers;
};

struct HtRange {
    explicit HtRange(const char *name);
    ~HtRange();
    bool on;
};

ht_status ht_fail(ht_ctx *ctx, ht_status st, const std::string &msg);
#define HT_HIP(ctx, call)                                                                                   \
    do {                                                                                                    \
        hipError_t e_ = (call);                                                                             \
        if (e_ != hipSuccess)                                                                               \
            return ht_fail((ctx), HT_ERR_HIP, std::string(#call) + ": " + hipGetErrorString(e_));           \
    } while (0)

template <typename T>
ht_status ht_grow_device(ht_ctx *c, T **p, size_t *cap, size_t need, const char *message) {
    if (*cap >= need) return HT_OK;
    HT_HIP(c, hipStreamSynchronize(c->stream));
    if (*p) (void)hipFree(*p);
    *p = nullptr, *cap = 0;
    if (hipMalloc(reinterpret_cast<void **>(p), need * sizeof(T)) != hipSuccess) {
        (void)hipGetLastError();
        return ht_fail(c, HT_ERR_NOMEM, message);
    }
    *cap = need;
    return HT_OK;
}

struct HtProfScope {
    ht_ctx *ctx;
    hipStream_t stream;
    int idx = -1;
    hipEvent_t a = nullptr, b = nullptr;
    HtProfScope(ht_ctx *c, const char *name, hipStream_t on = nullptr);
    ~HtProfScope();
};

void ht_capture_mark(ht_ctx *ctx, bool on);
ht_status ht_cs_hist_launch(ht_ctx *ctx, const uint8_t *frames, size_t frame_stride, int n, uint32_t npix, uint32_t chunk_px, uint32_t nchunks, uint32_t *hist);
ht_status ht_cs_ring_begin(ht_ctx *ctx, const char *fn, int32_t n, const ht_cs_trackobj *out, bool *via_ring, ht_ctx::HtCsSlot **slot);
void ht_cs_ring_commit(ht_ctx *ctx, ht_ctx::HtCsSlot *slot, int32_t n);
ht_status ht_cs_cluster_gate_begin(ht_ctx *ctx);
ht_status ht_cs_cluster_gate_end(ht_ctx *ctx);
ht_status ht_cs_check_err(ht_ctx *ctx, const char *where);
ht_status ht_cs_read_back(ht_ctx *ctx, const char *fn, ht_cs_trackobj *out, const ht_cs_trackobj *d_src, size_t count);
void ht_camshift_free(ht_ctx *ctx);
void ht_backproject_free(ht_ctx *ctx);
void ht_cs_pairs_free(ht_ctx *ctx);
void ht_cs_best_free(ht_ctx *ctx);
void ht_ingest_free(ht_ctx *ctx);
void ht_group_free(ht_ctx *ctx);
ht_status ht_detect_mark_collected(ht_ctx *ctx, bool wb_snap);
ht_status ht_frames_own_reserve(ht_ctx *ctx, size_t need, const char *fn);
void ht_frames_bind_own(ht_ctx *ctx, int n);
ht_status ht_launch_pyramid(ht_ctx *ctx, uint32_t flags);
ht_status ht_launch_scan(ht_ctx *ctx, uint32_t flags);
ht_status ht_launch_scan_early(ht_ctx *ctx, uint32_t flags);
bool ht_scan_is_builtin_cascade(const uint8_t *blob, size_t len);
ht_status ht_launch_gray_inplace(ht_ctx *ctx, uint8_t *d_rgba, int n, size_t stride);
ht_status ht_launch_whitebalance(ht_ctx *ctx, double *d_out, bool zero);
```

### headtrackr_amd/csrc/ht_plan_types.h

```cpp
#pragma once

#include <stdint.h>

#include <vector>

#include "headtrackr_hip.h"

struct HtDevLevel {
    int32_t w, h, stride;
    uint32_t off[4];
};

constexpr int HT_TAIL_MAX_GENS = 8;
constexpr int HT_TAIL_MAX_JOBS = 32;
struct HtTailGens {
    int32_t ngen;
    int32_t job_begin[HT_TAIL_MAX_GENS + 1];
    uint32_t groups[HT_TAIL_MAX_GENS];
    uint32_t tap_begin[HT_TAIL_MAX_GENS + 1];
};

struct HtTap {
    double t, u;
    int32_t a, b;
};
struct HtTapFast {
    int32_t a;
    float tf;
};
struct HtTailTapRef {
    uint32_t col, row;
    uint32_t mode;
    uint32_t pad;
};

constexpr int HT_RS_SRC_ROWS = 75;
constexpr int HT_RS_MAX_PASSES = 4;
struct HtResampleJob {
    uint32_t src_off, dst_off;
    int32_t src_stride, dst_stride;
    int32_t sx, sy, sw, sh;
    int32_t dw, dh;
    int32_t cw, ch;
    uint16_t bx, pass0;
    uint16_t np, pad;
    double rx, ry;
    int32_t ex_xa, ex_ya;
    int32_t ex_sw16, ex_sh;
    uint32_t band_ya4, band_sh4;
};
constexpr int HT_RSB_ROWS = 24;

constexpr int HT_SCAN_TXH = 64;
constexpr int HT_SCAN_TYH = 32;
struct HtScanScale {
    int32_t l0, l1, l2;
    int32_t qw, qh;
    int32_t tw2, th2;
    int32_t ntx, nty;
    uint32_t tile_begin;
    uint32_t div_magic;
    uint32_t win_begin;
};

struct alignas(64) HtTileRec {
    uint32_t off0, off1, off2[4];
    uint32_t sh0, sh1, sh2;
    uint32_t origin;
    uint32_t size;
    uint32_t tw2_l0;
    uint32_t div_magic;
    uint32_t strip_magic;
    uint32_t pad[2];
};
static_assert(sizeof(HtTileRec) == 64, "HtTileRec");

struct HtPlanInputs {
    int interval, next;
    uint32_t cw, ch;
    int rs_rpt;
    bool rs_nofast, rs_nosort, rs_notail;
    uint64_t rs_tailcap;
    bool rs_tailcap_forced;
    int tail_table;
    bool tail_table_forced;
    bool early_scan, aux_stream;
    uint32_t queue_capacity_cfg;
};

struct HtGeometryPlan {
    HtDevLevel levels[HT_MAX_LEVELS] = {};
    uint64_t arena_stride = 0;
    uint64_t pyr_bytes = 0, windows_per_frame = 0;
    std::vector<std::vector<HtResampleJob>> gens;
    std::vector<std::vector<HtResampleJob>> gen_tiles;
    std::vector<uint32_t> gen_blocks;
    int tail_first_gen = 0;
    int tail_table = 0;
    std::vector<HtResampleJob> tail_jobs;
    std::vector<uint32_t> tail_prefix;
    std::vector<HtTap> tail_taps;
    std::vector<HtTapFast> tail_taps_fast;
    std::vector<HtTailTapRef> tail_tapref;
    HtTailGens tail = {};
    std::vector<HtScanScale> scales;
    std::vector<HtTileRec> tile_recs;
    uint32_t tiles_per_frame = 0;
    int early_gen = 0;
    uint32_t early_tiles = 0;
    uint32_t queue_capacity = 0;
};
```

### headtrackr_amd/csrc/ht_pyramid.hip

```cpp
#include <cstdio>
#include <cstdlib>
#include <cstring>
#include <type_traits>

#include "ht_internal.h"
#include "ht_resample_tap.h"

namespace {

__device__ __forceinline__ bool xcd_item(uint32_t per_frame, uint32_t nframes, uint32_t *frame, uint32_t *item) {
    const uint32_t chunk = gridDim.x >> 3;
    const uint32_t t = (blockIdx.x & 7u) * chunk + (blockIdx.x >> 3);
    if (t >= per_frame * nframes) return false;
    *frame = t / per_frame;
    *item = t - *frame * per_frame;
    return true;
}

__device__ __forceinline__ uint32_t gray_of(uint32_t px) {
    const double r = (double)(px & 0xffu), g = (double)((px >> 8) & 0xffu), b = (double)((px >> 16) & 0xffu);
    const double v = __dadd_rn(__dadd_rn(__dmul_rn(r, 0.3), __dmul_rn(g, 0.59)), __dmul_rn(b, 0.11));
    const int q = (int)__builtin_rint(v);
    return (uint32_t)min(max(q, 0), 255);
}

template <bool GRAY_IN_R, bool WB>
__global__ __launch_bounds__(256) void k_gray_linear(const uint8_t *__restrict__ frames, size_t frame_stride,
                                                     uint8_t *__restrict__ arena, uint64_t arena_stride, uint32_t off0,
                                                     uint32_t ngroups, uint32_t blocks_per_frame, uint32_t nframes,
                                                     unsigned long long *__restrict__ wb_sums) {
    uint32_t f, blk;
    if (!xcd_item(blocks_per_frame, nframes, &f, &blk)) return;
    const uint4 *src = reinterpret_cast<const uint4 *>(frames + (size_t)f * frame_stride);
    uint32_t *dst = reinterpret_cast<uint32_t *>(arena + (uint64_t)f * arena_stride + off0);
    uint32_t sr = 0, sg = 0, sb = 0;
    for (uint32_t g = blk * blockDim.x + threadIdx.x; g < ngroups; g += blocks_per_frame * blockDim.x) {
        const uint4 p = src[g];
        uint32_t o;
        if (GRAY_IN_R)
            o = (p.x & 0xff) | ((p.y & 0xff) << 8) | ((p.z & 0xff) << 16) | ((p.w & 0xff) << 24);
        else
            o = gray_of(p.x) | (gray_of(p.y) << 8) | (gray_of(p.z) << 16) | (gray_of(p.w) << 24);
        dst[g] = o;
        if (WB) {
            const uint32_t rb = (p.x & 0x00ff00ffu) + (p.y & 0x00ff00ffu) + (p.z & 0x00ff00ffu) + (p.w & 0x00ff00ffu);
            sr += rb & 0xffffu;
            sb += rb >> 16;
            sg += ((p.x >> 8) & 0xffu) + ((p.y >> 8) & 0xffu) + ((p.z >> 8) & 0xffu) + ((p.w >> 8) & 0xffu);
        }
    }
    if (WB) {
        __shared__ uint32_t s_part[4][3];
#pragma unroll
        for (int s = 32; s > 0; s >>= 1) {
            sr += __shfl_xor(sr, s, 64);
            sg += __shfl_xor(sg, s, 64);
            sb += __shfl_xor(sb, s, 64);
        }
        if ((threadIdx.x & 63u) == 0) s_part[threadIdx.x >> 6][0] = sr, s_part[threadIdx.x >> 6][1] = sg, s_part[threadIdx.x >> 6][2] = sb;
        __syncthreads();
        if (threadIdx.x < 3) {
            const unsigned long long v = (unsigned long long)s_part[0][threadIdx.x] + s_part[1][threadIdx.x] + s_part[2][threadIdx.x] + s_part[3][threadIdx.x];
            atomicAdd(&wb_sums[(size_t)f * 4 + threadIdx.x], v);
        }
    }
}

template <bool GRAY_IN_R>
__global__ __launch_bounds__(256) void k_gray_rows(const uint8_t *__restrict__ frames, size_t frame_stride,
                                                   uint8_t *__restrict__ arena, uint64_t arena_stride, uint32_t off0, int W,
                                                   int H, int stride) {
    const uint32_t f = blockIdx.z;
    const int x0 = (blockIdx.x * 64 + threadIdx.x) * 4, y = blockIdx.y * 4 + threadIdx.y;
    if (y >= H || x0 >= stride) return;
    const uint32_t *src = reinterpret_cast<const uint32_t *>(frames + (size_t)f * frame_stride) + (size_t)y * W;
    uint32_t o = 0;
#pragma unroll
    for (int k = 0; k < 4; k++) {
        if (x0 + k < W) {
            const uint32_t p = src[x0 + k];
            o |= (GRAY_IN_R ? (p & 0xff) : gray_of(p)) << (8 * k);
        }
    }
    *reinterpret_cast<uint32_t *>(arena + (uint64_t)f * arena_stride + off0 + (size_t)y * stride + x0) = o;
}

__global__ __launch_bounds__(256) void k_gray_inplace(uint8_t *__restrict__ frames, size_t frame_stride, uint32_t npix) {
    uint32_t *p = reinterpret_cast<uint32_t *>(frames + (size_t)blockIdx.y * frame_stride);
    for (uint32_t i = blockIdx.x * blockDim.x + threadIdx.x; i < npix; i += gridDim.x * blockDim.x) {
        const uint32_t v = p[i], g = gray_of(v);
        p[i] = g | (g << 8) | (g << 16) | (v & 0xff000000u);
    }
}

constexpr int RS_TW = 64;
constexpr int RS_ROWB = 160;
constexpr int RS_SP = 160;
static_assert(RS_SP >= RS_ROWB && RS_SP % 16 == 0, "RS_SP");

typedef unsigned int rs_u32x4 __attribute__((ext_vector_type(4)));
typedef float rs_f2 __attribute__((ext_vector_type(2)));
__device__ __forceinline__ uint4 rs_buf_load16(__amdgpu_buffer_rsrc_t r, uint32_t voff, uint32_t soff) {
    const rs_u32x4 v = __builtin_amdgcn_raw_buffer_load_b128(r, voff, soff, 0);
    return make_uint4(v.x, v.y, v.z, v.w);
}

template <typename PTR>
__device__ __forceinline__ uint32_t rs_pixels4(PTR r0, PTR r1, const RsTap (&cx)[4], const RsTap &ry, int xoff, int npx) {
    uint32_t o = 0;
#pragma unroll
    for (int k = 0; k < 4; k++) {
        if (k < npx) {
            const int ia = cx[k].a - xoff, ib = cx[k].b - xoff;
            const double top = __dadd_rn(__dmul_rn((double)r0[ia], cx[k].u), __dmul_rn((double)r0[ib], cx[k].t));
            const double bot = __dadd_rn(__dmul_rn((double)r1[ia], cx[k].u), __dmul_rn((double)r1[ib], cx[k].t));
            const double vv = __dadd_rn(__dmul_rn(top, ry.u), __dmul_rn(bot, ry.t));
            const int q = (int)__builtin_rint(vv);
            o |= (uint32_t)q << (8 * k);
        }
    }
    return o;
}

#define RS_LDS_BARRIER()                                                     \
    do {                                                                     \
        __builtin_amdgcn_fence(__ATOMIC_RELEASE, "workgroup", "local");      \
        __builtin_amdgcn_s_barrier();                                        \
        __builtin_amdgcn_fence(__ATOMIC_ACQUIRE, "workgroup", "local");      \
    } while (0)
#define RS_LD1(ptr_) __hip_atomic_load((ptr_), __ATOMIC_RELAXED, __HIP_MEMORY_SCOPE_WORKGROUP)

__device__ __forceinline__ uint32_t rs_pixel_f64(const uint8_t *p, const uint8_t *p1, double cu, double ct, double ru, double rt) {
    const double top = __dadd_rn(__dmul_rn((double)p[0], cu), __dmul_rn((double)p1[0], ct));
    const double bot = __dadd_rn(__dmul_rn((double)p[RS_SP], cu), __dmul_rn((double)p1[RS_SP], ct));
    const double vv = __dadd_rn(__dmul_rn(top, ru), __dmul_rn(bot, rt));
    return (uint32_t)__double2loint(__dadd_rn(vv, 6755399441055744.0));
}

constexpr float RS_EPS = 1.0f / 8192.0f;

constexpr int RS_WPS = 6;
#if defined(HT_RS_PHASES)
__device__ unsigned long long g_rs_tl[16384][8][8];
__device__ unsigned long long g_rs_launch[1024][4];
__device__ unsigned long long g_rs_tw[4096][4][6];
#define RS_WSTAMP(i)                                                                                                                  \
    do {                                                                                                                              \
        __builtin_amdgcn_sched_barrier(0);                                                                                            \
        if (rs_iter == 2u && (threadIdx.x & 63u) == 0) g_rs_tw[rs_slot & 4095u][threadIdx.x >> 6][i] = __builtin_readcyclecounter(); \
        __builtin_amdgcn_sched_barrier(0);                                                                                            \
    } while (0)
#define HT_RS_TIMELINE 1
#define RS_SUB(i)                                                                       \
    do {                                                                                \
        __builtin_amdgcn_sched_barrier(0);                                              \
        if (threadIdx.x == 0) g_rs_tl[rs_slot][7][i] = __builtin_readcyclecounter();    \
        __builtin_amdgcn_sched_barrier(0);                                              \
    } while (0)
#define RS_STAMP(i)                                                                     \
    do {                                                                                \
        __builtin_amdgcn_sched_barrier(0);                                              \
        if (threadIdx.x == 0) g_rs_tl[rs_slot][rs_iter & 7u][i] = __builtin_readcyclecounter(); \
        __builtin_amdgcn_sched_barrier(0);                                              \
    } while (0)
#elif defined(HT_RS_TIMELINE)
__device__ unsigned long long g_rs_timeline[1 << 16][8];
#define RS_STAMP(i)                                                                     \
    do {                                                                                \
        __builtin_amdgcn_sched_barrier(0);                                              \
        if (threadIdx.x == 0) g_rs_timeline[blockIdx.x & 0xffffu][i] = __builtin_readcyclecounter(); \
        __builtin_amdgcn_sched_barrier(0);                                              \
    } while (0)
#else
#define RS_STAMP(i)
#endif
#ifndef RS_SUB
#define RS_SUB(i)
#endif
#ifndef RS_WSTAMP
#define RS_WSTAMP(i)
#endif
template <int RPT>
__global__ __launch_bounds__(256, RS_WPS) void k_resample(const HtResampleJob *__restrict__ tiles, uint8_t *__restrict__ arena,
                                                  uint64_t arena_stride, uint32_t blocks_per_frame, uint32_t ngroups,
                                                  uint32_t nframes, uint32_t group_frames) {
    constexpr int TH = 16 * RPT;
    constexpr int SR = HT_RS_SRC_ROWS;
    __shared__ __attribute__((aligned(16))) uint8_t s_src[(SR + 1) * RS_SP + 16];
    __shared__ RsTap s_col[RS_TW], s_row[TH];
    uint32_t gidx, blk;
    if (!xcd_item(blocks_per_frame, ngroups, &gidx, &blk)) return;
    __builtin_amdgcn_s_setprio(3);
#ifdef HT_RS_PHASES
    const uint32_t rs_slot = (blockIdx.x ^ (blocks_per_frame * 2654435761u)) & 16383u;
    uint32_t rs_iter = 0;
#endif
    RS_STAMP(0);
#ifdef HT_RS_PHASES
    const unsigned long long rs_t_entry = __builtin_readcyclecounter();
    auto rs_exit = [&]() {
        if (threadIdx.x == 0) {
            const unsigned long long now = __builtin_readcyclecounter();
            unsigned long long *L = g_rs_launch[blocks_per_frame & 1023u];
            atomicAdd(&L[0], 1ull);
            atomicAdd(&L[1], now - rs_t_entry);
        }
    };
#endif
    const HtResampleJob J = tiles[blk];
    const uint32_t f0 = gidx * group_frames, f1 = min(f0 + group_frames, nframes);
    const int tid = (int)threadIdx.x;
    const int np = (int)J.np;
    const int X0 = (int)J.bx * RS_TW, Y0 = (int)J.pass0 * 16;
    uint8_t *frame = arena + (uint64_t)f0 * arena_stride;
    const int ncols = min(RS_TW, J.dw - X0), nrows = min(16 * np, J.dh - Y0);
    const int x0 = X0 + (tid & 15) * 4, yt = Y0 + (tid >> 4);
    const int npx = min(4, J.dw - x0);
    const bool drawn = ncols > 0 && nrows > 0;
    RS_SUB(0);
    int xa = 0, ya = 0, sw16 = 1, sh = 1;
    bool in_lds = false;
    if (drawn) {
        if (J.ex_sw16 > 0) {
            xa = J.ex_xa, ya = J.ex_ya, sw16 = J.ex_sw16, sh = J.ex_sh;
        } else {
            xa = rs_tap(X0, J.rx, J.sw, J.sx).a & ~15;
            ya = rs_tap(Y0, J.ry, J.sh, J.sy).a;
            sw16 = (rs_tap(X0 + ncols - 1, J.rx, J.sw, J.sx).b - xa) / 16 + 1;
            sh = rs_tap(Y0 + nrows - 1, J.ry, J.sh, J.sy).b - ya + 1;
        }
        xa = __builtin_amdgcn_readfirstlane(xa), ya = __builtin_amdgcn_readfirstlane(ya);
        sw16 = __builtin_amdgcn_readfirstlane(sw16), sh = __builtin_amdgcn_readfirstlane(sh);
        in_lds = (sw16 * 16 <= RS_ROWB) && (sh <= SR);
    }
    RS_SUB(1);
    if (in_lds) {
        constexpr int KR = (SR + 24) / 25;
        static_assert(KR == 3, "the staging registers below are written out for three passes");
        const int r0 = (tid * 205) >> 11, c16 = tid - r0 * 10;
        const bool lane_on = (r0 < 25) && (c16 < sw16);
        const uint32_t soff = J.src_off + (uint32_t)(ya * J.src_stride + xa + 16 * min(c16, sw16 - 1));
        const uint32_t soff0 = soff + (uint32_t)(min(r0, sh - 1) * J.src_stride), soff1 = soff + (uint32_t)(min(r0 + 25, sh - 1) * J.src_stride);
        const uint32_t soff2 = soff + (uint32_t)(min(r0 + 50, sh - 1) * J.src_stride);
        uint8_t *const sdst = &s_src[r0 * RS_SP + 16 * c16];
        const bool w0on = lane_on && r0 < sh, w1on = lane_on && r0 + 25 < sh, w2on = lane_on && r0 + 50 < sh;
        uint64_t fbase = reinterpret_cast<uint64_t>(frame);
#define RS_FRAME_RSRC(base_) __builtin_amdgcn_make_buffer_rsrc(reinterpret_cast<void *>(base_), 0, (int)0xffffffffu, 0x00020000)
#define RS_TILE_TO_LDS()                                                          \
    do {                                                                          \
        if (w0on) *reinterpret_cast<uint4 *>(sdst) = v0;                          \
        if (w1on) *reinterpret_cast<uint4 *>(sdst + 25 * RS_SP) = v1;             \
        if (w2on) *reinterpret_cast<uint4 *>(sdst + 50 * RS_SP) = v2;             \
    } while (0)
        RS_SUB(2);
        {
            const __amdgpu_buffer_rsrc_t fr = RS_FRAME_RSRC(fbase);
            const uint4 v0 = rs_buf_load16(fr, soff0, 0u), v1 = rs_buf_load16(fr, soff1, 0u), v2 = rs_buf_load16(fr, soff2, 0u);
            RS_SUB(3);
            if (tid < ncols) s_col[tid] = rs_tap(X0 + tid, J.rx, J.sw, J.sx);
            if (tid >= 64 && tid - 64 < nrows) s_row[tid - 64] = rs_tap(Y0 + tid - 64, J.ry, J.sh, J.sy);
            RS_SUB(4);
            RS_TILE_TO_LDS();
        }
        __syncthreads();
        __builtin_amdgcn_s_setprio(0);
        RS_STAMP(1);
        const int cbase = x0 - X0;
        int ia[4];
        float ctf[4];
#pragma unroll
        for (int k = 0; k < 4; k++) {
            const RsTap *ct = &s_col[min(cbase + k, ncols - 1)];
            ia[k] = ct->a - xa, ctf[k] = (float)ct->t;
        }
        uint32_t one = 1u;
        asm volatile("" : "+s"(one));
        const uint32_t mode = J.pad;
        const float thr = (mode & 2u) ? -1.0f : 0.5f - RS_EPS;
        const int dh = J.dh, ch = J.ch, dst_stride = J.dst_stride;
        const uint32_t doff = J.dst_off + (uint32_t)(yt * dst_stride + x0);
        const uint32_t pxmask = npx >= 4 ? 0xffffffffu : (npx <= 0 ? 0u : ((1u << (8 * npx)) - 1u));
        const int ia8 = npx > 0 ? ia[0] : 0;
        auto frames = [&](auto NPc, auto BOXc) {
            constexpr int NP = decltype(NPc)::value;
            constexpr bool BOX = decltype(BOXc)::value;
            uint32_t roff[NP];
            float rtf[NP];
            bool st[NP], rv[NP];
#pragma unroll
            for (int q = 0; q < NP; q++) {
                const int y = yt + 16 * q;
                const RsTap *ry = &s_row[min(y - Y0, nrows - 1)];
                roff[q] = (uint32_t)((ry->a - ya) * RS_SP);
                rtf[q] = (float)ry->t;
                rv[q] = y < dh;
                st[q] = y < ch && x0 < dst_stride;
            }
            for (uint32_t f = f0; f < f1; f++) {
                asm volatile("" : "+s"(fbase));
                const __amdgpu_buffer_rsrc_t fr = RS_FRAME_RSRC(fbase);
                fbase += arena_stride;
#pragma unroll
                for (int q = 0; q < NP; q++) asm volatile("" : "+v"(roff[q]));
                RS_STAMP(2);
                uint4 v0, v1, v2;
                if (f + 1 < f1) {
                    v0 = rs_buf_load16(fr, soff0, (uint32_t)arena_stride);
                    v1 = rs_buf_load16(fr, soff1, (uint32_t)arena_stride);
                    v2 = rs_buf_load16(fr, soff2, (uint32_t)arena_stride);
                }
                RS_STAMP(3);
                RS_WSTAMP(0);
                uint32_t o[NP];
                if (BOX) {
#pragma unroll
                    for (int q = 0; q < NP; q++) {
                        const uint8_t *row = s_src + roff[q] + ia8;
                        const uint2 A = *reinterpret_cast<const uint2 *>(row), B = *reinterpret_cast<const uint2 *>(row + RS_SP);
                        uint32_t oq = 0;
#pragma unroll
                        for (int k = 0; k < 4; k++) {
                            const uint32_t a = k < 2 ? A.x : A.y, b = k < 2 ? B.x : B.y;
                            const uint32_t g = __builtin_amdgcn_perm(b, a, (k & 1) ? 0x07060302u : 0x05040100u);
                            const uint32_t sum = __builtin_amdgcn_sad_u8(g, 0u, 0u);
                            oq = __builtin_amdgcn_cvt_pk_u8_f32(__builtin_rintf((float)sum * 0.25f), k, oq);
                        }
                        o[q] = rv[q] ? (oq & pxmask) : 0u;
                    }
                } else {
                    uint32_t T[16];
#pragma unroll
                    for (int q = 0; q < NP; q++) {
                        const uint8_t *row_ = s_src + roff[q];
#pragma unroll
                        for (int k = 0; k < 4; k++) {
                            const uint8_t *p_ = row_ + ia[k];
                            T[4 * k] = p_[0], T[4 * k + 1] = RS_LD1(p_ + 1), T[4 * k + 2] = p_[RS_SP], T[4 * k + 3] = RS_LD1(p_ + RS_SP + 1);
                        }
                        __builtin_amdgcn_sched_barrier(0);
                        float d[4];
                        uint32_t oq = 0;
#pragma unroll
                        for (int k = 0; k < 4; k++) {
                            const float p00 = (float)T[4 * k], p01 = (float)T[4 * k + 1], p10 = (float)T[4 * k + 2], p11 = (float)T[4 * k + 3];
                            const rs_f2 lo2 = {p00, p10}, hi2 = {p01, p11}, ct2 = {ctf[k], ctf[k]};
                            const rs_f2 tb = __builtin_elementwise_fma(ct2, hi2 - lo2, lo2);
                            const float top = tb.x, bot = tb.y;
                            const float v = __builtin_fmaf(rtf[q], bot - top, top);
                            const float r = __builtin_rintf(v);
                            d[k] = v - r;
                            oq = __builtin_amdgcn_cvt_pk_u8_f32(r, k, oq);
                        }
                        const float dmq = __builtin_fmaxf(__builtin_fmaxf(__builtin_fabsf(d[0]), __builtin_fabsf(d[1])), __builtin_fmaxf(__builtin_fabsf(d[2]), __builtin_fabsf(d[3])));
                        if (dmq >= thr) {
                            uint32_t roff_f = roff[q];
                            int yrel = yt - Y0, cb = cbase;
                            asm volatile("" : "+v"(roff_f), "+v"(yrel), "+v"(cb));
                            const RsTap *ry = &s_row[min(yrel + 16 * q, nrows - 1)];
                            const uint8_t *rowf = s_src + roff_f;
#pragma unroll
                            for (int k = 0; k < 4; k++) {
                                if (__builtin_fabsf(d[k]) >= thr) {
                                    const RsTap *ct = &s_col[min(cb + k, ncols - 1)];
                                    oq &= ~(0xffu << (8 * k));
                                    oq |= rs_pixel_f64(rowf + ia[k], rowf + ia[k] + one, ct->u, ct->t, ry->u, ry->t) << (8 * k);
                                }
                            }
                        }
                        o[q] = rv[q] ? (oq & pxmask) : 0u;
                    }
                }
#ifdef HT_RS_TIMELINE
#pragma unroll
                for (int q = 0; q < NP; q++) asm volatile("" ::"v"(o[q]));
                RS_STAMP(4);
                RS_WSTAMP(1);
#endif
#define RS_WRITE_ROWS()                                                                                                                             \
    _Pragma("unroll") for (int q = 0; q < NP; q++) if (st[q])                                                                                      \
        __builtin_amdgcn_raw_buffer_store_b32(o[q], fr, doff, (uint32_t)(16 * q * dst_stride), 0)
                if (f + 1 < f1) {
                    RS_LDS_BARRIER();
                    RS_STAMP(5);
                    RS_WSTAMP(2);
                    RS_TILE_TO_LDS();
                    RS_WRITE_ROWS();
                    RS_LDS_BARRIER();
                    RS_WSTAMP(3);
#ifdef HT_RS_PHASES
                    if (rs_iter == 2u && (threadIdx.x & 63u) == 0) g_rs_tw[rs_slot & 4095u][threadIdx.x >> 6][4] = __builtin_amdgcn_s_getreg((4 << 0) | (0 << 6) | (31 << 11));
#endif
                } else {
                    RS_WRITE_ROWS();
                    RS_STAMP(5);
                }
#undef RS_WRITE_ROWS
                RS_STAMP(6);
#ifdef HT_RS_PHASES
                rs_iter++;
#endif
            }
        };
        using std::integral_constant;
        if (mode & 1u) {
            switch (np) {
                case 1: frames(integral_constant<int, 1>{}, integral_constant<bool, true>{}); break;
                case 2: frames(integral_constant<int, 2>{}, integral_constant<bool, true>{}); break;
                case 3: frames(integral_constant<int, 3>{}, integral_constant<bool, true>{}); break;
                default: frames(integral_constant<int, RPT>{}, integral_constant<bool, true>{}); break;
            }
        } else {
            switch (np) {
                case 1: frames(integral_constant<int, 1>{}, integral_constant<bool, false>{}); break;
                case 2: frames(integral_constant<int, 2>{}, integral_constant<bool, false>{}); break;
                case 3: frames(integral_constant<int, 3>{}, integral_constant<bool, false>{}); break;
                default: frames(integral_constant<int, RPT>{}, integral_constant<bool, false>{}); break;
            }
        }
#undef RS_TILE_TO_LDS
#undef RS_FRAME_RSRC
#ifdef HT_RS_PHASES
        rs_exit();
#endif
        return;
    }
    const HtResampleJob &Jm = tiles[blk];
    RsTap cx[4];
#pragma unroll
    for (int k = 0; k < 4; k++) cx[k] = rs_tap(min(x0 + k, X0 + max(ncols, 1) - 1), Jm.rx, Jm.sw, Jm.sx);
    for (uint32_t f = f0; f < f1; f++, frame += arena_stride) {
        const uint8_t *src = frame + Jm.src_off;
        int ytl = yt;
        asm volatile("" : "+v"(ytl));
#pragma unroll
        for (int q = 0; q < RPT; q++) {
            const int y = ytl + 16 * q;
            uint32_t o = 0;
            if (drawn && q < np && y < Jm.dh && npx > 0) {
                const RsTap ry = rs_tap(y, Jm.ry, Jm.sh, Jm.sy);
                o = rs_pixels4<const uint8_t *>(src + (size_t)ry.a * Jm.src_stride, src + (size_t)ry.b * Jm.src_stride, cx, ry, 0, npx);
            }
            if (q < np && y < Jm.ch && x0 < Jm.dst_stride) *reinterpret_cast<uint32_t *>(frame + Jm.dst_off + (size_t)y * Jm.dst_stride + x0) = o;
        }
    }
}

constexpr int RSB_WPS = 8;
constexpr int RSB_BAND = 4096;
#if defined(HT_RS_PHASES)
__device__ unsigned long long g_rsb_ph[256][8];
#define RSB_T(var_)                                     \
    do {                                                \
        __builtin_amdgcn_sched_barrier(0);              \
        var_ = __builtin_readcyclecounter();            \
        __builtin_amdgcn_sched_barrier(0);              \
    } while (0)
#else
#define RSB_T(var_)
#endif
typedef __attribute__((address_space(3))) void rs_lds_void;
template <int RPT>
__global__ __launch_bounds__(256, RSB_WPS) void k_resample_bands(const HtResampleJob *__restrict__ tiles, uint8_t *__restrict__ arena,
                                                                    uint64_t arena_stride, uint32_t blocks_per_frame, uint32_t ngroups,
                                                                    uint32_t nframes, uint32_t group_frames) {
    constexpr int TH = 16 * RPT;
    __shared__ __attribute__((aligned(16))) uint8_t s_src[4 * RSB_BAND];
    __shared__ RsTap s_col[RS_TW], s_row[TH];
    uint32_t gidx, blk;
    if (!xcd_item(blocks_per_frame, ngroups, &gidx, &blk)) return;
#ifdef HT_RS_PHASES
    unsigned long long rsb_t_entry = 0, rsb_t0 = 0, rsb_t1 = 0, rsb_t2 = 0, rsb_t3 = 0, rsb_t4 = 0, rsb_acc[7] = {0, 0, 0, 0, 0, 0, 0};
    RSB_T(rsb_t_entry);
#endif
    const HtResampleJob J = tiles[blk];
    const uint32_t f0 = gidx * group_frames, f1 = min(f0 + group_frames, nframes);
    const int tid = (int)threadIdx.x;
    const int np = (int)J.np;
    const int X0 = (int)J.bx * RS_TW, Y0 = (int)J.pass0 * 16;
    uint8_t *frame = arena + (uint64_t)f0 * arena_stride;
    const int ncols = min(RS_TW, J.dw - X0), nrows = min(16 * np, J.dh - Y0);
    const uint32_t mode = J.pad;
    if ((mode & 4u) && ncols > 0 && nrows > 0) {
        const int w = __builtin_amdgcn_readfirstlane(tid >> 6), l = tid & 63;
        const int xa = J.ex_xa, sw16 = J.ex_sw16;
        const int yaw = J.ex_ya + (int)((J.band_ya4 >> (8 * w)) & 0xffu);
        const int bsh = (int)((J.band_sh4 >> (8 * w)) & 0xffu);
        uint8_t *const band = s_src + w * RSB_BAND;
        uint32_t voff[4];
        bool on[4];
#pragma unroll
        for (int i = 0; i < 4; i++) {
            const int c = i * 64 + l, row = (c * 205) >> 11, col = c - row * 10;
            on[i] = col < sw16 && row < bsh;
            voff[i] = J.src_off + (uint32_t)((yaw + row) * J.src_stride + xa + 16 * col);
        }
        uint64_t fbase = reinterpret_cast<uint64_t>(frame);
#define RS_FRAME_RSRC(base_) __builtin_amdgcn_make_buffer_rsrc(reinterpret_cast<void *>(base_), 0, (int)0xffffffffu, 0x00020000)
#define RSB_DMA(fr_, soff_)                                                                                                              \
    do {                                                                                                                                 \
        _Pragma("unroll") for (int i = 0; i < 4; i++) if (on[i])                                                                         \
            __builtin_amdgcn_raw_ptr_buffer_load_lds(fr_, (rs_lds_void *)(band + i * 1024), 16, voff[i], soff_, 0, 0);                   \
    } while (0)
        {
            const __amdgpu_buffer_rsrc_t fr = RS_FRAME_RSRC(fbase);
            RSB_DMA(fr, 0u);
            if (tid < ncols) s_col[tid] = rs_tap(X0 + tid, J.rx, J.sw, J.sx);
            if (tid >= 64 && tid - 64 < nrows) s_row[tid - 64] = rs_tap(Y0 + tid - 64, J.ry, J.sh, J.sy);
        }
        __syncthreads();
        const int cbase = (l & 15) * 4, x0 = X0 + cbase;
        const int yt = Y0 + 4 * np * w + (l >> 4);
        const int npx = min(4, J.dw - x0);
        int ia[4];
        float ctf[4];
#pragma unroll
        for (int k = 0; k < 4; k++) {
            const RsTap *ct = &s_col[min(cbase + k, ncols - 1)];
            ia[k] = ct->a - xa, ctf[k] = (float)ct->t;
        }
        uint32_t one = 1u;
        asm volatile("" : "+s"(one));
        const float thr = (mode & 2u) ? -1.0f : 0.5f - RS_EPS;
        const int dh = J.dh, ch = J.ch, dst_stride = J.dst_stride;
        const uint32_t doff = J.dst_off + (uint32_t)(yt * dst_stride + x0);
        const uint32_t pxmask = npx >= 4 ? 0xffffffffu : (npx <= 0 ? 0u : ((1u << (8 * npx)) - 1u));
        const int ia8 = npx > 0 ? ia[0] : 0;
        auto frames = [&](auto NPc, auto BOXc) {
            constexpr int NP = decltype(NPc)::value;
            constexpr bool BOX = decltype(BOXc)::value;
            uint32_t roff[NP];
            float rtf[NP];
            bool st[NP], rv[NP];
#pragma unroll
            for (int q = 0; q < NP; q++) {
                const int y = yt + 4 * q;
                const RsTap *ry = &s_row[min(y - Y0, nrows - 1)];
                roff[q] = (uint32_t)((ry->a - yaw) * RS_SP + w * RSB_BAND);
                rtf[q] = (float)ry->t;
                rv[q] = y < dh;
                st[q] = y < ch && x0 < dst_stride;
            }
            for (uint32_t f = f0; f < f1; f++) {
                asm volatile("" : "+s"(fbase));
                const __amdgpu_buffer_rsrc_t fr = RS_FRAME_RSRC(fbase);
                fbase += arena_stride;
#pragma unroll
                for (int q = 0; q < NP; q++) asm volatile("" : "+v"(roff[q]));
#ifdef HT_RS_PHASES
                if (f == f0 && w == 0) rsb_acc[5] = 1ull, rsb_acc[6] = __builtin_readcyclecounter() - rsb_t_entry;
#endif
                RSB_T(rsb_t0);
                uint32_t o[NP];
                if (BOX) {
#pragma unroll
                    for (int q = 0; q < NP; q++) {
                        const uint8_t *row = s_src + roff[q] + ia8;
                        const uint2 A = *reinterpret_cast<const uint2 *>(row), B = *reinterpret_cast<const uint2 *>(row + RS_SP);
                        uint32_t oq = 0;
#pragma unroll
                        for (int k = 0; k < 4; k++) {
                            const uint32_t a = k < 2 ? A.x : A.y, b = k < 2 ? B.x : B.y;
                            const uint32_t g = __builtin_amdgcn_perm(b, a, (k & 1) ? 0x07060302u : 0x05040100u);
                            const uint32_t sum = __builtin_amdgcn_sad_u8(g, 0u, 0u);
                            oq = __builtin_amdgcn_cvt_pk_u8_f32(__builtin_rintf((float)sum * 0.25f), k, oq);
                        }
                        o[q] = rv[q] ? (oq & pxmask) : 0u;
                    }
                } else {
                    uint32_t T[16];
#pragma unroll
                    for (int q = 0; q < NP; q++) {
                        const uint8_t *row_ = s_src + roff[q];
#pragma unroll
                        for (int k = 0; k < 4; k++) {
                            const uint8_t *p_ = row_ + ia[k];
                            T[4 * k] = p_[0], T[4 * k + 1] = RS_LD1(p_ + 1), T[4 * k + 2] = p_[RS_SP], T[4 * k + 3] = RS_LD1(p_ + RS_SP + 1);
                        }
                        __builtin_amdgcn_sched_barrier(0);
                        float d[4];
                        uint32_t oq = 0;
#pragma unroll
                        for (int k = 0; k < 4; k++) {
                            const float p00 = (float)T[4 * k], p01 = (float)T[4 * k + 1], p10 = (float)T[4 * k + 2], p11 = (float)T[4 * k + 3];
                            const rs_f2 lo2 = {p00, p10}, hi2 = {p01, p11}, ct2 = {ctf[k], ctf[k]};
                            const rs_f2 tb = __builtin_elementwise_fma(ct2, hi2 - lo2, lo2);
                            const float top = tb.x, bot = tb.y;
                            const float v = __builtin_fmaf(rtf[q], bot - top, top);
                            const float r = __builtin_rintf(v);
                            d[k] = v - r;
                            oq = __builtin_amdgcn_cvt_pk_u8_f32(r, k, oq);
                        }
                        const float dmq = __builtin_fmaxf(__builtin_fmaxf(__builtin_fabsf(d[0]), __builtin_fabsf(d[1])), __builtin_fmaxf(__builtin_fabsf(d[2]), __builtin_fabsf(d[3])));
                        if (dmq >= thr) {
                            uint32_t roff_f = roff[q];
                            int yrel = yt - Y0, cb = cbase;
                            asm volatile("" : "+v"(roff_f), "+v"(yrel), "+v"(cb));
                            const RsTap *ry = &s_row[min(yrel + 4 * q, nrows - 1)];
                            const uint8_t *rowf = s_src + roff_f;
#pragma unroll
                            for (int k = 0; k < 4; k++) {
                                if (__builtin_fabsf(d[k]) >= thr) {
                                    const RsTap *ct = &s_col[min(cb + k, ncols - 1)];
                                    oq &= ~(0xffu << (8 * k));
                                    oq |= rs_pixel_f64(rowf + ia[k], rowf + ia[k] + one, ct->u, ct->t, ry->u, ry->t) << (8 * k);
                                }
                            }
                        }
                        o[q] = rv[q] ? (oq & pxmask) : 0u;
                    }
                }
#ifdef HT_RS_PHASES
#pragma unroll
                for (int q = 0; q < NP; q++) asm volatile("" ::"v"(o[q]));
#endif
                RSB_T(rsb_t1);
                if (f + 1 < f1) {
                    __builtin_amdgcn_s_waitcnt(0xc07f);
                    RSB_DMA(fr, (uint32_t)arena_stride);
                    RSB_T(rsb_t2);
                    __builtin_amdgcn_s_waitcnt(0x0f70);
                    RSB_T(rsb_t3);
                }
#pragma unroll
                for (int q = 0; q < NP; q++)
                    if (st[q]) __builtin_amdgcn_raw_buffer_store_b32(o[q], fr, doff, (uint32_t)(4 * q * dst_stride), 0);
#ifdef HT_RS_PHASES
                RSB_T(rsb_t4);
                if (f + 1 < f1) {
                    rsb_acc[0] += 1ull, rsb_acc[1] += rsb_t1 - rsb_t0, rsb_acc[2] += rsb_t2 - rsb_t1, rsb_acc[3] += rsb_t3 - rsb_t2, rsb_acc[4] += rsb_t4 - rsb_t3;
                }
#endif
            }
#ifdef HT_RS_PHASES
            if (l == 0) {
#pragma unroll
                for (int i = 0; i < 7; i++)
                    if (rsb_acc[i]) atomicAdd(&g_rsb_ph[blockIdx.x & 255u][i], rsb_acc[i]);
            }
#endif
        };
        using std::integral_constant;
        if (mode & 1u) {
            switch (np) {
                case 1: frames(integral_constant<int, 1>{}, integral_constant<bool, true>{}); break;
                case 2: frames(integral_constant<int, 2>{}, integral_constant<bool, true>{}); break;
                case 3: frames(integral_constant<int, 3>{}, integral_constant<bool, true>{}); break;
                default: frames(integral_constant<int, RPT>{}, integral_constant<bool, true>{}); break;
            }
        } else {
            switch (np) {
                case 1: frames(integral_constant<int, 1>{}, integral_constant<bool, false>{}); break;
                case 2: frames(integral_constant<int, 2>{}, integral_constant<bool, false>{}); break;
                case 3: frames(integral_constant<int, 3>{}, integral_constant<bool, false>{}); break;
                default: frames(integral_constant<int, RPT>{}, integral_constant<bool, false>{}); break;
            }
        }
#undef RSB_DMA
#undef RS_FRAME_RSRC
        return;
    }
    const HtResampleJob &Jm = tiles[blk];
    const int x0 = X0 + (tid & 15) * 4, yt = Y0 + (tid >> 4);
    const int npx = min(4, Jm.dw - x0);
    const bool drawn = ncols > 0 && nrows > 0;
    RsTap cx[4];
#pragma unroll
    for (int k = 0; k < 4; k++) cx[k] = rs_tap(min(x0 + k, X0 + max(ncols, 1) - 1), Jm.rx, Jm.sw, Jm.sx);
    for (uint32_t f = f0; f < f1; f++, frame += arena_stride) {
        const uint8_t *src = frame + Jm.src_off;
        int ytl = yt;
        asm volatile("" : "+v"(ytl));
#pragma unroll
        for (int q = 0; q < RPT; q++) {
            const int y = ytl + 16 * q;
            uint32_t o = 0;
            if (drawn && q < np && y < Jm.dh && npx > 0) {
                const RsTap ry = rs_tap(y, Jm.ry, Jm.sh, Jm.sy);
                o = rs_pixels4<const uint8_t *>(src + (size_t)ry.a * Jm.src_stride, src + (size_t)ry.b * Jm.src_stride, cx, ry, 0, npx);
            }
            if (q < np && y < Jm.ch && x0 < Jm.dst_stride) *reinterpret_cast<uint32_t *>(frame + Jm.dst_off + (size_t)y * Jm.dst_stride + x0) = o;
        }
    }
}

constexpr int TAIL_NT = 1024;
constexpr int TAIL_U = 1;
constexpr int TAIL_SMALL_WPS = 8;
template <bool LDS_TAPS, int WPS>
__global__ __launch_bounds__(TAIL_NT, WPS) void k_resample_tail(const HtResampleJob *__restrict__ jobs, const uint32_t *__restrict__ prefix,
                                                          const HtTailTapRef *__restrict__ tapref, const HtTapFast *__restrict__ tfast,
                                                          const HtTap *__restrict__ tfull, const HtTailGens G, uint8_t *__restrict__ arena,
                                                          uint64_t arena_stride, uint32_t nframes) {
    __shared__ HtResampleJob s_jobs[HT_TAIL_MAX_JOBS];
    __shared__ HtTailTapRef s_ref[HT_TAIL_MAX_JOBS];
    __shared__ uint32_t s_pref[HT_TAIL_MAX_JOBS + 1];
    __shared__ HtTapFast s_taps[LDS_TAPS ? HT_TAIL_LDS_TAPS : 1];
    uint32_t fidx, item;
    if (!xcd_item(1u, nframes, &fidx, &item)) return;
    uint8_t *frame = arena + (uint64_t)fidx * arena_stride;
    const int tid = (int)threadIdx.x;
    for (int g = 0; g < G.ngen; g++) {
        const int jb = G.job_begin[g], nj = G.job_begin[g + 1] - jb;
        const uint32_t total = G.groups[g];
        {
            const uint32_t *src32 = reinterpret_cast<const uint32_t *>(jobs + jb);
            uint32_t *dst32 = reinterpret_cast<uint32_t *>(s_jobs);
            for (int i = tid; i < nj * (int)(sizeof(HtResampleJob) / 4); i += TAIL_NT) dst32[i] = src32[i];
            if (tid < nj) s_pref[tid] = prefix[jb + tid], s_ref[tid] = tapref[jb + tid];
            if (tid == 0) s_pref[nj] = total;
        }
        const uint32_t tap0 = G.tap_begin[g], ntap = G.tap_begin[g + 1] - tap0;
        const bool taps_in_lds = LDS_TAPS && ntap <= (uint32_t)HT_TAIL_LDS_TAPS;
        if (taps_in_lds)
            for (uint32_t i = (uint32_t)tid; i < ntap; i += TAIL_NT) s_taps[i] = tfast[tap0 + i];
        __syncthreads();
        for (uint32_t i0 = (uint32_t)tid; i0 < total; i0 += TAIL_U * TAIL_NT) {
            bool live[TAIL_U], draw[TAIL_U];
            uint32_t doff[TAIL_U], mode[TAIL_U], tcol[TAIL_U], trow[TAIL_U];
            int npx[TAIL_U], sstride[TAIL_U], dwm1[TAIL_U];
            const uint8_t *sbase[TAIL_U];
#pragma unroll
            for (int u = 0; u < TAIL_U; u++) {
                const uint32_t i = i0 + u * TAIL_NT;
                live[u] = i < total;
                const uint32_t ii = live[u] ? i : 0u;
                int lo = 0, hi = nj;
                while (hi - lo > 1) {
                    const int mid = (lo + hi) >> 1;
                    if (s_pref[mid] <= ii) lo = mid;
                    else hi = mid;
                }
                const HtResampleJob &J = s_jobs[lo];
                const HtTailTapRef ref = s_ref[lo];
                const uint32_t q = ii - s_pref[lo], qpr = (uint32_t)(J.cw + 3) >> 2;
                const uint32_t y = q / qpr, x0 = (q - y * qpr) * 4u;
                npx[u] = min(4, J.dw - (int)x0);
                draw[u] = live[u] && (int)y < J.dh && npx[u] > 0;
                doff[u] = J.dst_off + y * (uint32_t)J.dst_stride + x0;
                mode[u] = ref.mode;
                tcol[u] = ref.col + (draw[u] ? x0 : 0u);
                trow[u] = ref.row + (draw[u] ? y : 0u);
                sstride[u] = J.src_stride;
                sbase[u] = frame + J.src_off;
                dwm1[u] = max(J.dw - 1 - (int)x0, 0);
            }
            HtTapFast ctap[TAIL_U][4], rtap[TAIL_U];
#pragma unroll
            for (int u = 0; u < TAIL_U; u++) {
                if (taps_in_lds) {
                    const HtTapFast *cf = s_taps + (tcol[u] - tap0);
                    ctap[u][0] = cf[0], ctap[u][1] = cf[1], ctap[u][2] = cf[2], ctap[u][3] = cf[3];
                    rtap[u] = s_taps[trow[u] - tap0];
                } else {
                    const HtTapFast *cf = tfast + tcol[u];
                    ctap[u][0] = cf[0], ctap[u][1] = cf[1], ctap[u][2] = cf[2], ctap[u][3] = cf[3];
                    rtap[u] = tfast[trow[u]];
                }
            }
            uint32_t p00[TAIL_U][4], p01[TAIL_U][4], p10[TAIL_U][4], p11[TAIL_U][4];
#pragma unroll
            for (int u = 0; u < TAIL_U; u++) {
                const uint8_t *r0 = sbase[u] + (size_t)rtap[u].a * sstride[u], *r1 = r0 + (rtap[u].tf != 0.0f ? sstride[u] : 0);
#pragma unroll
                for (int k = 0; k < 4; k++) {
                    const int ca = ctap[u][k].a, cb = ca + (ctap[u][k].tf != 0.0f ? 1 : 0);
                    p00[u][k] = r0[ca], p01[u][k] = r0[cb], p10[u][k] = r1[ca], p11[u][k] = r1[cb];
                }
            }
#pragma unroll
            for (int u = 0; u < TAIL_U; u++) {
                uint32_t o = 0;
                if (draw[u]) {
                    auto exact64 = [&](int k) {
                        const HtTap cx = tfull[tcol[u] + min(k, dwm1[u])], ry = tfull[trow[u]];
                        const uint8_t *s0 = sbase[u] + (size_t)ry.a * sstride[u], *s1 = sbase[u] + (size_t)ry.b * sstride[u];
                        const double top = __dadd_rn(__dmul_rn((double)s0[cx.a], cx.u), __dmul_rn((double)s0[cx.b], cx.t));
                        const double bot = __dadd_rn(__dmul_rn((double)s1[cx.a], cx.u), __dmul_rn((double)s1[cx.b], cx.t));
                        const double vv = __dadd_rn(__dmul_rn(top, ry.u), __dmul_rn(bot, ry.t));
                        return (uint32_t)(int)__builtin_rint(vv);
                    };
                    uint32_t need = 0, obox = 0;
#pragma unroll
                    for (int k = 0; k < 4; k++) {
                        const uint32_t sum = p00[u][k] + p01[u][k] + p10[u][k] + p11[u][k], qq = sum >> 2, r4 = sum & 3u;
                        obox |= (qq + ((r4 + (qq & 1u)) > 2u ? 1u : 0u)) << (8 * k);
                        const float a00 = (float)p00[u][k], a10 = (float)p10[u][k];
                        const float top = __builtin_fmaf(ctap[u][k].tf, (float)p01[u][k] - a00, a00);
                        const float bot = __builtin_fmaf(ctap[u][k].tf, (float)p11[u][k] - a10, a10);
                        const float v = __builtin_fmaf(rtap[u].tf, bot - top, top);
                        const float r = __builtin_rintf(v);
                        if (__builtin_fabsf(v - r) >= 0.5f - RS_EPS) need |= 1u << k;
                        o |= (uint32_t)(int)r << (8 * k);
                    }
                    const uint32_t keep = npx[u] >= 4 ? 0xffffffffu : ((1u << (8 * npx[u])) - 1u);
                    if (mode[u] & 1u) o = obox, need = 0;
                    if (mode[u] & 2u) need = 0xfu;
                    need &= (1u << npx[u]) - 1u;
                    o &= keep;
                    if (need) {
#pragma unroll
                        for (int k = 0; k < 4; k++)
                            if (need & (1u << k)) o = (o & ~(0xffu << (8 * k))) | (exact64(k) << (8 * k));
                    }
                }
                if (live[u]) *reinterpret_cast<uint32_t *>(frame + doff[u]) = o;
            }
        }
        __syncthreads();
    }
}

constexpr int TAILF_NT = 1024;
__global__ __launch_bounds__(TAILF_NT) void k_resample_tail_f64(const HtResampleJob *__restrict__ jobs, const uint32_t *__restrict__ prefix,
                                                          const HtTailGens G, uint8_t *__restrict__ arena, uint64_t arena_stride,
                                                          uint32_t nframes) {
    __shared__ HtResampleJob s_jobs[HT_TAIL_MAX_JOBS];
    __shared__ uint32_t s_pref[HT_TAIL_MAX_JOBS + 1];
    uint32_t fidx, item;
    if (!xcd_item(1u, nframes, &fidx, &item)) return;
    uint8_t *frame = arena + (uint64_t)fidx * arena_stride;
    const int tid = (int)threadIdx.x;
    for (int g = 0; g < G.ngen; g++) {
        const int jb = G.job_begin[g], nj = G.job_begin[g + 1] - jb;
        const uint32_t total = G.groups[g];
        {
            const uint32_t *src32 = reinterpret_cast<const uint32_t *>(jobs + jb);
            uint32_t *dst32 = reinterpret_cast<uint32_t *>(s_jobs);
            for (int i = tid; i < nj * (int)(sizeof(HtResampleJob) / 4); i += TAILF_NT) dst32[i] = src32[i];
            if (tid < nj) s_pref[tid] = prefix[jb + tid];
            if (tid == 0) s_pref[nj] = total;
        }
        __syncthreads();
        for (uint32_t i = (uint32_t)tid; i < total; i += TAILF_NT) {
            int lo = 0, hi = nj;
            while (hi - lo > 1) {
                const int mid = (lo + hi) >> 1;
                if (s_pref[mid] <= i) lo = mid;
                else hi = mid;
            }
            const HtResampleJob &J = s_jobs[lo];
            const uint32_t q = i - s_pref[lo], qpr = (uint32_t)(J.cw + 3) >> 2;
            const uint32_t y = q / qpr, x0 = (q - y * qpr) * 4u;
            uint32_t o = 0;
            const int npx = min(4, J.dw - (int)x0);
            if ((int)y < J.dh && npx > 0) {
                const uint8_t *src = frame + J.src_off;
                RsTap cx[4];
#pragma unroll
                for (int k = 0; k < 4; k++) cx[k] = rs_tap(min((int)x0 + k, J.dw - 1), J.rx, J.sw, J.sx);
                const RsTap ry = rs_tap((int)y, J.ry, J.sh, J.sy);
                o = rs_pixels4<const uint8_t *>(src + (size_t)ry.a * J.src_stride, src + (size_t)ry.b * J.src_stride, cx, ry, 0, npx);
            }
            *reinterpret_cast<uint32_t *>(frame + J.dst_off + (size_t)y * J.dst_stride + x0) = o;
        }
        __syncthreads();
    }
}

__global__ __launch_bounds__(256) void k_channel_sums(const uint8_t *__restrict__ frames, size_t frame_stride, uint32_t npix,
                                                      unsigned long long *__restrict__ out) {
    const uint32_t *p = reinterpret_cast<const uint32_t *>(frames + (size_t)blockIdx.y * frame_stride);
    uint32_t r = 0, g = 0, b = 0;
    for (uint32_t i = blockIdx.x * blockDim.x + threadIdx.x; i < npix; i += gridDim.x * blockDim.x) {
        const uint32_t v = p[i];
        r += v & 0xff;
        g += (v >> 8) & 0xff;
        b += (v >> 16) & 0xff;
    }
    unsigned long long rr = r, gg = g, bb = b;
#pragma unroll
    for (int s = 32; s > 0; s >>= 1) {
        rr += __shfl_xor(rr, s, 64);
        gg += __shfl_xor(gg, s, 64);
        bb += __shfl_xor(bb, s, 64);
    }
    if ((threadIdx.x & 63) == 0) {
        atomicAdd(&out[blockIdx.y * 4 + 0], rr);
        atomicAdd(&out[blockIdx.y * 4 + 1], gg);
        atomicAdd(&out[blockIdx.y * 4 + 2], bb);
    }
}

}

ht_status ht_launch_pyramid(ht_ctx *c, uint32_t flags) {
    const bool gray_in_r = (flags & HT_INPUT_GRAY_IN_R) != 0;
    const HtDevLevel &L0 = c->plan.levels[0];
    {
        HtProfScope ps(c, "gray");
        if ((c->W & 3) == 0) {
            const uint32_t ngroups = (uint32_t)((size_t)c->W * c->H / 4);
            const uint32_t bpf = std::min<uint32_t>((ngroups + 255) / 256, 2048);
            dim3 grid((bpf * (uint32_t)c->nframes + 7u) & ~7u);
            unsigned long long *wb = c->wb_fused ? reinterpret_cast<unsigned long long *>(c->d_scratch) : nullptr;
#define HT_GRAY_LAUNCH(G, W_)                                                                                                          \
    hipLaunchKernelGGL((k_gray_linear<G, W_>), grid, dim3(256), 0, c->stream, c->d_frames, c->frame_stride, c->d_arena, c->plan.arena_stride, \
                       L0.off[0], ngroups, bpf, (uint32_t)c->nframes, wb)
            if (gray_in_r) {
                if (wb) HT_GRAY_LAUNCH(true, true);
                else HT_GRAY_LAUNCH(true, false);
            } else {
                if (wb) HT_GRAY_LAUNCH(false, true);
                else HT_GRAY_LAUNCH(false, false);
            }
#undef HT_GRAY_LAUNCH
        } else {
            dim3 grid((L0.stride / 4 + 63) / 64, (c->H + 3) / 4, c->nframes);
            if (gray_in_r)
                hipLaunchKernelGGL(k_gray_rows<true>, grid, dim3(64, 4), 0, c->stream, c->d_frames, c->frame_stride, c->d_arena,
                                   c->plan.arena_stride, L0.off[0], c->W, c->H, L0.stride);
            else
                hipLaunchKernelGGL(k_gray_rows<false>, grid, dim3(64, 4), 0, c->stream, c->d_frames, c->frame_stride, c->d_arena,
                                   c->plan.arena_stride, L0.off[0], c->W, c->H, L0.stride);
        }
        HT_HIP(c, hipGetLastError());
    }
    const size_t regular_end = c->plan.tail_first_gen > 0 ? (size_t)c->plan.tail_first_gen : c->plan.gens.size();
    const int dbg_maxgen = c->rs_maxgen;
    for (size_t g = 1; g < regular_end; g++) {
        if (c->plan.gen_blocks[g] == 0 || (int)g > dbg_maxgen) continue;
        char gname[24];
        std::snprintf(gname, sizeof(gname), "resample_g%d", (int)g);
        HtProfScope ps(c, c->rs_gennames ? gname : "resample");
        uint32_t K = 1;
        const uint32_t kmax = (uint32_t)((!c->rs_group_forced && (int64_t)c->W * c->H >= 400000) ? std::min(c->rs_group, 4) : c->rs_group);
        while (K * 2 <= kmax && (uint64_t)c->plan.gen_blocks[g] * ((uint32_t)c->nframes / (K * 2)) >= (uint64_t)c->rs_min_wgs &&
               (uint32_t)c->nframes % (K * 2 * 8) == 0)
            K *= 2;
        if (c->dbg_rs_k > 0) K = (uint32_t)std::min(c->dbg_rs_k, std::max(1, c->nframes));
        const uint32_t ngroups = ((uint32_t)c->nframes + K - 1) / K;
        const dim3 rgrid((c->plan.gen_blocks[g] * ngroups + 7u) & ~7u);
        if (c->rs_bands)
            hipLaunchKernelGGL(k_resample_bands<HT_RS_MAX_PASSES>, rgrid, dim3(256), 0, c->stream, c->d_gen_blocks[g], c->d_arena, c->plan.arena_stride,
                               c->plan.gen_blocks[g], ngroups, (uint32_t)c->nframes, K);
        else
            hipLaunchKernelGGL(k_resample<HT_RS_MAX_PASSES>, rgrid, dim3(256), 0, c->stream, c->d_gen_blocks[g], c->d_arena, c->plan.arena_stride,
                               c->plan.gen_blocks[g], ngroups, (uint32_t)c->nframes, K);
        HT_HIP(c, hipGetLastError());
        if ((int)g == c->plan.early_gen && c->plan.early_gen > 0) {
            ht_status st = ht_launch_scan_early(c, flags);
            if (st != HT_OK) return st;
        }
    }
    if (c->plan.tail_first_gen > 0 && c->plan.tail_first_gen <= dbg_maxgen) {
        HtProfScope ps(c, c->rs_gennames ? "resample_tail" : "resample");
        if (c->plan.tail_table == 2)
            hipLaunchKernelGGL((k_resample_tail<false, TAIL_SMALL_WPS>), dim3(((uint32_t)c->nframes + 7u) & ~7u), dim3(TAIL_NT), 0, c->stream, c->d_tail_jobs,
                               c->d_tail_prefix, c->d_tail_tapref, c->d_tail_taps_fast, c->d_tail_taps, c->plan.tail, c->d_arena, c->plan.arena_stride, (uint32_t)c->nframes);
        else if (c->plan.tail_table)
            hipLaunchKernelGGL((k_resample_tail<true, 4>), dim3(((uint32_t)c->nframes + 7u) & ~7u), dim3(TAIL_NT), 0, c->stream, c->d_tail_jobs, c->d_tail_prefix,
                               c->d_tail_tapref, c->d_tail_taps_fast, c->d_tail_taps, c->plan.tail, c->d_arena, c->plan.arena_stride, (uint32_t)c->nframes);
        else
            hipLaunchKernelGGL(k_resample_tail_f64, dim3(((uint32_t)c->nframes + 7u) & ~7u), dim3(TAILF_NT), 0, c->stream, c->d_tail_jobs, c->d_tail_prefix,
                               c->plan.tail, c->d_arena, c->plan.arena_stride, (uint32_t)c->nframes);
        HT_HIP(c, hipGetLastError());
    }
    return HT_OK;
}

ht_status ht_launch_gray_inplace(ht_ctx *c, uint8_t *d_rgba, int n, size_t stride) {
    HtProfScope ps(c, "gray_inplace");
    const uint32_t npix = (uint32_t)((size_t)c->W * c->H);
    hipLaunchKernelGGL(k_gray_inplace, dim3(std::min<uint32_t>((npix + 255) / 256, 2048), n), dim3(256), 0, c->stream, d_rgba, stride, npix);
    HT_HIP(c, hipGetLastError());
    return HT_OK;
}

ht_status ht_launch_whitebalance(ht_ctx *c, double *d_out, bool zero) {
    HtProfScope ps(c, "whitebalance");
    unsigned long long *out = reinterpret_cast<unsigned long long *>(d_out);
    if (zero) HT_HIP(c, hipMemsetAsync(out, 0, sizeof(unsigned long long) * 4 * (size_t)c->nframes, c->stream));
    const uint32_t npix = (uint32_t)((size_t)c->W * c->H);
    hipLaunchKernelGGL(k_channel_sums, dim3(std::min<uint32_t>((npix + 1023) / 1024, 256), c->nframes), dim3(256), 0, c->stream,
                       c->d_frames, c->frame_stride, npix, out);
    HT_HIP(c, hipGetLastError());
    return HT_OK;
}

#ifdef HT_RS_PHASES
extern "C" int ht_debug_rsb_phases(unsigned long long *out8, int reset) {
    static unsigned long long h[256][8];
    if (hipMemcpyFromSymbol(h, HIP_SYMBOL(g_rsb_ph), sizeof(h)) != hipSuccess) return 1;
    for (int i = 0; i < 8; i++) out8[i] = 0;
    for (int sh = 0; sh < 256; sh++)
        for (int i = 0; i < 8; i++) out8[i] += h[sh][i];
    if (reset) {
        std::memset(h, 0, sizeof(h));
        if (hipMemcpyToSymbol(HIP_SYMBOL(g_rsb_ph), h, sizeof(h)) != hipSuccess) return 1;
    }
    return 0;
}
extern "C" int ht_debug_rs_phases(unsigned long long *out16, int reset) {
    static unsigned long long h[16384][8][8];
    if (hipMemcpyFromSymbol(h, HIP_SYMBOL(g_rs_tl), sizeof(h)) != hipSuccess) return 1;
    for (int j = 0; j < 16; j++) out16[j] = 0;
    for (int sl = 0; sl < 16384; sl++)
        for (int it = 0; it < 8; it++) {
            const unsigned long long *t = h[sl][it];
            if (!t[2] || !t[6] || t[6] < t[2] || t[6] - t[2] > (1ull << 18) || t[3] < t[2] || t[4] < t[3] || t[5] < t[4] || t[6] < t[5]) continue;
            for (int i = 3; i <= 6; i++) out16[i] += t[i] - t[i - 1], out16[8 + i]++;
            if (it == 0 && h[sl][0][0] && h[sl][0][0] <= h[sl][0][1] && h[sl][0][1] <= t[2] && t[2] - h[sl][0][0] < (1ull << 16)) {
                out16[1] += h[sl][0][1] - h[sl][0][0], out16[8 + 1]++;
                out16[2] += t[2] - h[sl][0][1], out16[8 + 2]++;
            }
        }
    if (const char *e = std::getenv("HT_RS_SUBSTAMPS")) {
        (void)e;
        unsigned long long sum[6] = {}, n = 0;
        for (int sl = 0; sl < 16384; sl++) {
            const unsigned long long *u = h[sl][7], t0 = h[sl][0][0], t1 = h[sl][0][1];
            if (!t0 || !t1 || !u[0] || !u[4] || t1 < t0 || t1 - t0 > (1ull << 24) || u[0] < t0 || u[4] > t1) continue;
            sum[0] += u[0] - t0, sum[1] += u[1] - u[0], sum[2] += u[2] - u[1], sum[3] += u[3] - u[2], sum[4] += u[4] - u[3], sum[5] += t1 - u[4], n++;
        }
        if (n) std::printf("  setup sub-phases (%llu samples): record %.0f, extents %.0f, addresses %.0f, load issue %.0f, tap tables %.0f, barrier %.0f cycles\n", n,
                           (double)sum[0] / n, (double)sum[1] / n, (double)sum[2] / n, (double)sum[3] / n, (double)sum[4] / n, (double)sum[5] / n);
    }
    if (std::getenv("HT_RS_LAUNCHES")) {
        static unsigned long long L[1024][4];
        if (hipMemcpyFromSymbol(L, HIP_SYMBOL(g_rs_launch), sizeof(L)) != hipSuccess) return 1;
        for (int k = 0; k < 1024; k++)
            if (L[k][0]) std::printf("  launches with %4d tiles per frame: %6llu workgroups (LDS path), mean life %7.0f cycles\n", k, L[k][0], (double)L[k][1] / (double)L[k][0]);
    }
    if (std::getenv("HT_RS_WAVESTAMPS")) {
        static unsigned long long w[4096][4][6];
        if (hipMemcpyFromSymbol(w, HIP_SYMBOL(g_rs_tw), sizeof(w)) != hipSuccess) return 1;
        double pix[4] = {}, wait1[4] = {}, mid[4] = {}, spread = 0, pixmax = 0, pixmin = 0;
        unsigned long long n = 0, simd_hist[4][4] = {};
        for (int sl = 0; sl < 4096; sl++) {
            bool ok = true;
            unsigned long long bmin = ~0ull, bmax = 0, pmn = ~0ull, pmx = 0;
            for (int k = 0; k < 4; k++) {
                const unsigned long long *t = w[sl][k];
                if (!t[0] || t[1] < t[0] || t[2] < t[1] || t[3] < t[2] || t[3] - t[0] > (1ull << 22)) ok = false;
                bmin = std::min(bmin, t[1]), bmax = std::max(bmax, t[1]);
                pmn = std::min(pmn, t[1] - t[0]), pmx = std::max(pmx, t[1] - t[0]);
            }
            if (!ok) continue;
            n++;
            spread += (double)(bmax - bmin), pixmax += (double)pmx, pixmin += (double)pmn;
            for (int k = 0; k < 4; k++) {
                const unsigned long long *t = w[sl][k];
                pix[k] += (double)(t[1] - t[0]), wait1[k] += (double)(t[2] - t[1]), mid[k] += (double)(t[3] - t[2]);
                simd_hist[k][(t[4] >> 4) & 3]++;
            }
        }
        if (n) {
            std::printf("  per-wave view (%llu workgroups, third frame iteration): pixel phase / wait at barrier 1 / tile write + stores + barrier 2, cycles\n", n);
            for (int k = 0; k < 4; k++)
                std::printf("    wave %d: %7.0f %7.0f %7.0f   SIMD histogram %llu %llu %llu %llu\n", k, pix[k] / n, wait1[k] / n, mid[k] / n, simd_hist[k][0], simd_hist[k][1],
                            simd_hist[k][2], simd_hist[k][3]);
            std::printf("    pixel phase of the fastest / slowest wave of a workgroup: %.0f / %.0f; spread of their arrival at barrier 1: %.0f cycles\n", pixmin / n, pixmax / n, spread / n);
        }
    }
    if (reset) {
        std::memset(h, 0, sizeof(h));
        if (hipMemcpyToSymbol(HIP_SYMBOL(g_rs_tl), h, sizeof(h)) != hipSuccess) return 1;
        static unsigned long long wz[4096][4][6];
        if (hipMemcpyToSymbol(HIP_SYMBOL(g_rs_tw), wz, sizeof(wz)) != hipSuccess) return 1;
        static unsigned long long lz[1024][4];
        for (int k = 0; k < 1024; k++) lz[k][0] = lz[k][1] = lz[k][3] = 0, lz[k][2] = ~0ull;
        if (hipMemcpyToSymbol(HIP_SYMBOL(g_rs_launch), lz, sizeof(lz)) != hipSuccess) return 1;
    }
    return 0;
}
#endif
```

Measured before the change: 1.165 million frames/s.

## Prune unused pyramid planes and add dense-tile resample layout for small frames

Adds a planning pass that marks which pyramid level/slot planes the scan actually reads, moves resample jobs for unused planes into a deferred set, and trims empty generations. The deferred planes are only built lazily when a pyramid readback asks for them. It also adds a dense tile layout for the banded resample kernel at small resolutions, packing several rows per wave with precomputed tap tables so fewer lanes idle on narrow levels. This adds complexity and a lazy-build path on readback, and taps are recomputed per pixel in the dense fallback path.

```diff
diff --git a/headtrackr_amd/csrc/ht_context.hip b/headtrackr_amd/csrc/ht_context.hip
--- a/headtrackr_amd/csrc/ht_context.hip
+++ b/headtrackr_amd/csrc/ht_context.hip
@@ -161,6 +161,8 @@
         else if (key == "rs_nofast") c->rs_nofast = iv != 0;
         else if (key == "rs_nosort") c->rs_nosort = iv != 0;
         else if (key == "rs_bands") c->rs_bands = iv != 0;
+        else if (key == "rs_dense") c->rs_dense = iv != 0;
+        else if (key == "rs_prune") c->rs_prune = iv != 0;
         else if (key == "rs_gennames") c->rs_gennames = iv != 0;
         else if (key == "rs_minwg") c->rs_min_wgs = std::max(1, iv);
         else if (key == "rs_k") c->dbg_rs_k = iv;
@@ -304,6 +306,20 @@
     for (auto p : c->d_gen_blocks)
         if (p) (void)hipFree(p);
     c->d_gen_blocks.clear();
+    for (auto p : c->d_dense_tiles)
+        if (p) (void)hipFree(p);
+    c->d_dense_tiles.clear();
+    for (auto p : c->d_dense_taps)
+        if (p) (void)hipFree(p);
+    c->d_dense_taps.clear();
+    c->plan.dense_tiles.clear();
+    c->plan.dense_taps.clear();
+    for (auto p : c->d_pruned_tiles)
+        if (p) (void)hipFree(p);
+    c->d_pruned_tiles.clear();
+    c->plan.pruned_gens.clear();
+    c->plan.pruned_tiles.clear();
+    c->pruned_built = false;
     if (c->d_tile_recs) (void)hipFree(c->d_tile_recs), c->d_tile_recs = nullptr;
     if (c->d_tail_jobs) (void)hipFree(c->d_tail_jobs), c->d_tail_jobs = nullptr;
     if (c->d_tail_prefix) (void)hipFree(c->d_tail_prefix), c->d_tail_prefix = nullptr;
@@ -395,6 +411,8 @@
     in.tail_table = c->tail_table, in.tail_table_forced = c->tail_table_forced;
     in.early_scan = c->early_scan, in.aux_stream = c->aux_stream != nullptr;
     in.queue_capacity_cfg = c->queue_capacity_cfg;
+    in.rs_dense = c->rs_bands && (c->rs_dense > 0 || (c->rs_dense < 0 && (int64_t)width * height < 400000));
+    in.rs_prune = c->rs_prune;
     HtGeometryPlan &P = c->plan;
     std::string why;
     ht_status st = ht_plan_geometry(in, width, height, max_batch, level_dims, n, upto, &P, &why);
@@ -403,6 +421,10 @@
     c->d_gen_blocks.assign(P.gens.size(), nullptr);
     for (size_t g = 1; g < P.gens.size(); g++)
         if ((st = upload_table(c, c->d_gen_blocks[g], P.gen_tiles[g])) != HT_OK) return st;
+    c->d_dense_tiles.assign(P.dense_tiles.size(), nullptr);
+    c->d_dense_taps.assign(P.dense_taps.size(), nullptr);
+    for (size_t g = 1; g < P.dense_tiles.size(); g++)
+        if ((st = upload_table(c, c->d_dense_tiles[g], P.dense_tiles[g])) != HT_OK || (st = upload_table(c, c->d_dense_taps[g], P.dense_taps[g])) != HT_OK) return st;
     HT_HIP(c, hipMalloc(&c->d_levels, sizeof(HtDevLevel) * HT_MAX_LEVELS));
     HT_HIP(c, hipMemcpy(c->d_levels, P.levels, sizeof(HtDevLevel) * n, hipMemcpyHostToDevice));
     if (hipMalloc(&c->d_arena, P.arena_stride * (uint64_t)max_batch) != hipSuccess)
@@ -747,6 +769,7 @@
     c->stats_enqueued = (flags & HT_SCAN_STATS) != 0;
     c->wb_enqueued = (flags & HT_DETECT_WHITEBALANCE) != 0;
     c->enqueued = true;
+    c->pruned_built = false;
     c->grp_enqueued = false;
     c->enq_nframes = c->nframes;
     return HT_OK;
@@ -873,6 +896,16 @@
     if (cap < (size_t)L.w * L.h) return ht_fail(c, HT_ERR_CAPACITY, "ht_pyramid_readback: buffer too small");
     if (L.w == 0 || L.h == 0) return HT_OK;
     HT_HIP(c, hipSetDevice(c->device));
+    if (!c->pruned_built && c->enq_nframes > 0) {
+        bool pruned = false;
+        for (auto &gen : c->plan.pruned_gens)
+            for (auto &j : gen) pruned = pruned || j.dst_off == L.off[slot];
+        if (pruned) {
+            const ht_status st = ht_launch_pruned_planes(c, c->enq_nframes);
+            if (st != HT_OK) return st;
+            c->pruned_built = true;
+        }
+    }
     HT_HIP(c, hipStreamSynchronize(c->stream));
     HT_HIP(c, hipMemcpy2D(out, L.w, c->d_arena + (uint64_t)frame * c->plan.arena_stride + L.off[slot], L.stride, L.w, L.h, hipMemcpyDeviceToHost));
     return HT_OK;
diff --git a/headtrackr_amd/csrc/ht_geometry_plan.h b/headtrackr_amd/csrc/ht_geometry_plan.h
--- a/headtrackr_amd/csrc/ht_geometry_plan.h
+++ b/headtrackr_amd/csrc/ht_geometry_plan.h
@@ -61,7 +61,7 @@
     return HT_OK;
 }
 
-static void ht_plan_jobs(const HtPlanInputs &in, int n, HtGeometryPlan *p, std::vector<int> &gen) {
+static void ht_plan_jobs(const HtPlanInputs &in, int n, int upto, HtGeometryPlan *p, std::vector<int> &gen) {
     const int next = in.next;
     gen.assign(n, 0);
     int ngen = 1;
@@ -70,6 +70,18 @@
         ngen = std::max(ngen, gen[i] + 1);
     }
     p->gens.assign(ngen, {});
+    std::vector<uint8_t> need((size_t)n * 4, in.rs_prune ? 0 : 1);
+    if (in.rs_prune) {
+        p->pruned_gens.assign(ngen, {});
+        for (int i = 0; i < upto; i++) {
+            const int l2 = i + 2 * next;
+            if (p->levels[l2].w - (int)(in.cw / 4) <= 0 || p->levels[l2].h - (int)(in.ch / 4) <= 0) continue;
+            need[4 * i] = need[4 * (i + next)] = 1;
+            for (int s = 0; s < 4; s++) need[4 * l2 + s] = 1;
+        }
+        for (int i = n - 1; i >= 1; i--)
+            if (need[4 * i] || need[4 * i + 1] || need[4 * i + 2] || need[4 * i + 3]) need[4 * (i <= in.interval ? 0 : i - next)] = 1;
+    }
     auto add_job = [&](int g, int src, int dst, int slot, int sx, int sy, int sw, int sh, int dw, int dh) {
         const HtDevLevel &S = p->levels[src], &D = p->levels[dst];
         if (D.w <= 0 || D.h <= 0) return;
@@ -90,7 +102,7 @@
             j.rx = (double)sw / (double)dw;
             j.ry = (double)sh / (double)dh;
         }
-        p->gens[g].push_back(j);
+        (need[4 * dst + slot] ? p->gens[g] : p->pruned_gens[g]).push_back(j);
     };
     for (int i = 1; i < n; i++) {
         const HtDevLevel &D = p->levels[i];
@@ -106,6 +118,8 @@
             }
         }
     }
+    if (in.rs_prune)
+        while (p->gens.size() > 1 && p->gens.back().empty()) p->gens.pop_back();
 }
 
 static std::vector<HtResampleJob> ht_plan_gen_tiles(const HtPlanInputs &in, const std::vector<HtResampleJob> &jobs) {
@@ -153,6 +167,106 @@
     return tiles;
 }
 
+static void ht_plan_dense_tiles(const HtPlanInputs &in, const std::vector<HtResampleJob> &jobs, std::vector<HtDenseTile> *tiles_out,
+                                std::vector<HtTapFast> *taps_out) {
+    std::vector<HtDenseTile> &tiles = *tiles_out;
+    tiles.clear(), taps_out->clear();
+    const int npcap = std::min(std::max(in.rs_rpt, 1), HT_RS_MAX_PASSES);
+    struct Strip {
+        int R, npmax, passes, tiles;
+    };
+    for (auto &j : jobs) {
+        auto band_rows = [&](int rows) { return (int)std::ceil((double)(rows - 1) * j.ry) + 2; };
+        auto plan_strip = [&](int ncg) {
+            Strip best = {0, 1, 0, 0};
+            int best_tiles = 0;
+            for (int R = 64 / ncg; R >= 1; R--) {
+                if (R > 1 && band_rows(R) > HT_RSB_ROWS) continue;
+                Strip s = {R, 1, (j.ch + 4 * R - 1) / (4 * R), 0};
+                for (int t = 2; t <= npcap; t++)
+                    if (band_rows(R * t) <= HT_RSB_ROWS) s.npmax = t;
+                const int ntiles = (s.passes + s.npmax - 1) / s.npmax;
+                if (!best.R || s.passes + ntiles < best.passes + best_tiles) best = s, best_tiles = ntiles;
+            }
+            best.tiles = best_tiles;
+            return best;
+        };
+        const int NCG = (j.cw + 3) / 4, nb0 = (NCG + 15) / 16;
+        int nbx = nb0, cost = 0;
+        for (int nb = nb0; nb <= std::min(NCG, nb0 + 2); nb++) {
+            int c = 0;
+            for (int x = 0; x < nb; x++) {
+                const Strip s = plan_strip(NCG / nb + (x < NCG % nb ? 1 : 0));
+                c += s.passes + s.tiles;
+            }
+            if (nb == nb0 || c < cost) nbx = nb, cost = c;
+        }
+        int cg0 = 0;
+        for (int x = 0; x < nbx; x++) {
+            const int ncg = NCG / nbx + (x < NCG % nbx ? 1 : 0);
+            const Strip s = plan_strip(ncg);
+            const int nby = (s.passes + s.npmax - 1) / s.npmax;
+            int pass0 = 0;
+            for (int y = 0; y < nby; y++) {
+                const int np = s.passes / nby + (y < s.passes % nby ? 1 : 0);
+                HtDenseTile t;
+                std::memset(&t, 0, sizeof(t));
+                t.src_off = j.src_off, t.dst_off = j.dst_off, t.src_stride = j.src_stride, t.dst_stride = j.dst_stride;
+                t.sx = j.sx, t.sy = j.sy, t.sw = j.sw, t.sh = j.sh, t.dw = j.dw, t.dh = j.dh, t.cw = j.cw, t.ch = j.ch;
+                t.rx = j.rx, t.ry = j.ry;
+                t.X0 = 4 * cg0, t.Y0 = 4 * s.R * pass0;
+                t.ncg = (uint16_t)ncg, t.R = (uint16_t)s.R, t.np = (uint16_t)np;
+                t.lane_magic = (65536u + (uint32_t)ncg - 1u) / (uint32_t)ncg;
+                t.mode = in.rs_nofast ? 2 : (uint16_t)((j.dw > 0 && j.sw == 2 * j.dw && j.sh == 2 * j.dh) ? 1 : 0);
+                const int rpw = s.R * np;
+                const int ncols = std::min(4 * ncg, j.dw - t.X0), nrows = std::min(4 * rpw, j.dh - t.Y0);
+                if (ncols > 0 && nrows > 0) {
+                    t.ex_xa = ht_host_tap(t.X0, j.rx, j.sw, j.sx).a & ~15;
+                    t.ex_ya = ht_host_tap(t.Y0, j.ry, j.sh, j.sy).a;
+                    t.ex_sw16 = (ht_host_tap(t.X0 + ncols - 1, j.rx, j.sw, j.sx).b - t.ex_xa) / 16 + 1;
+                    t.ex_sh = ht_host_tap(t.Y0 + nrows - 1, j.ry, j.sh, j.sy).b - t.ex_ya + 1;
+                    bool fit = t.ex_sw16 * 16 <= 160;
+                    for (int w = 0; w < 4; w++) {
+                        const int r0 = std::min(rpw * w, nrows - 1), r1 = std::min(rpw * (w + 1) - 1, nrows - 1);
+                        const int bya = ht_host_tap(t.Y0 + r0, j.ry, j.sh, j.sy).a - t.ex_ya;
+                        const int bsh = ht_host_tap(t.Y0 + r1, j.ry, j.sh, j.sy).b - (t.ex_ya + bya) + 1;
+                        if (bya < 0 || bya > 255 || bsh < 1 || bsh > HT_RSB_ROWS) fit = false;
+                        t.band_ya4 |= (uint32_t)(bya & 0xff) << (8 * w), t.band_sh4 |= (uint32_t)(bsh & 0xff) << (8 * w);
+                    }
+                    if (fit) t.mode |= 4;
+                }
+                tiles.push_back(t);
+                pass0 += np;
+            }
+            cg0 += ncg;
+        }
+    }
+    if (!in.rs_nosort)
+        std::stable_sort(tiles.begin(), tiles.end(), [](const HtDenseTile &a, const HtDenseTile &b) {
+            if (a.src_off != b.src_off) return a.src_off < b.src_off;
+            const int ya = (int)((double)a.Y0 * a.ry), yb = (int)((double)b.Y0 * b.ry);
+            if (ya / 32 != yb / 32) return ya < yb;
+            return a.X0 < b.X0;
+        });
+    std::vector<HtTapFast> &taps = *taps_out;
+    for (auto &t : tiles) {
+        if (!(t.mode & 4)) continue;
+        const int rpw = t.R * t.np;
+        const int ncols = std::min(4 * t.ncg, t.dw - t.X0), nrows = std::min(4 * rpw, t.dh - t.Y0);
+        t.tap_col = (uint32_t)taps.size();
+        for (int k = 0; k < 4 * t.ncg; k++) {
+            const HtTap c = ht_host_tap(t.X0 + std::min(k, ncols - 1), t.rx, t.sw, t.sx);
+            taps.push_back(HtTapFast{c.a - t.ex_xa, (float)c.t});
+        }
+        t.tap_row = (uint32_t)taps.size();
+        for (int i = 0; i < 4 * rpw; i++) {
+            const HtTap r = ht_host_tap(t.Y0 + std::min(i, nrows - 1), t.ry, t.sh, t.sy);
+            const int bya = (int)((t.band_ya4 >> (8 * (i / rpw))) & 0xffu);
+            taps.push_back(HtTapFast{r.a - (t.ex_ya + bya), (float)r.t});
+        }
+    }
+}
+
 static void ht_plan_tail(const HtPlanInputs &in, int max_batch, HtGeometryPlan *p) {
     const int ngen = (int)p->gens.size();
     constexpr int HT_SMALL_BATCH = 48;
@@ -293,7 +407,7 @@
     ht_status st = ht_plan_levels(in, width, height, level_dims, n, plan, why);
     if (st != HT_OK) return st;
     std::vector<int> gen;
-    ht_plan_jobs(in, n, plan, gen);
+    ht_plan_jobs(in, n, upto, plan, gen);
     const int ngen = (int)plan->gens.size();
     plan->gen_tiles.assign(ngen, {});
     plan->gen_blocks.assign(ngen, 0);
@@ -301,7 +415,15 @@
         plan->gen_tiles[g] = ht_plan_gen_tiles(in, plan->gens[g]);
         plan->gen_blocks[g] = (uint32_t)plan->gen_tiles[g].size();
     }
+    plan->pruned_tiles.assign(plan->pruned_gens.size(), {});
+    for (size_t g = 1; g < plan->pruned_gens.size(); g++) plan->pruned_tiles[g] = ht_plan_gen_tiles(in, plan->pruned_gens[g]);
     ht_plan_tail(in, max_batch, plan);
+    if (in.rs_dense) {
+        plan->dense_tiles.assign(ngen, {});
+        plan->dense_taps.assign(ngen, {});
+        const int regular_end = plan->tail_first_gen > 0 ? plan->tail_first_gen : ngen;
+        for (int g = 1; g < regular_end; g++) ht_plan_dense_tiles(in, plan->gens[g], &plan->dense_tiles[g], &plan->dense_taps[g]);
+    }
     if ((st = ht_plan_scan_tiles(in, upto, plan, why)) != HT_OK) return st;
     ht_plan_early_split(in, gen, plan);
     uint64_t qc = in.queue_capacity_cfg ? in.queue_capacity_cfg : std::max<uint64_t>(1u << 16, plan->windows_per_frame * (uint64_t)max_batch / 8);
diff --git a/headtrackr_amd/csrc/ht_internal.h b/headtrackr_amd/csrc/ht_internal.h
--- a/headtrackr_amd/csrc/ht_internal.h
+++ b/headtrackr_amd/csrc/ht_internal.h
@@ -92,6 +92,10 @@
     HtDevLevel *d_levels = nullptr;
     uint8_t *d_arena = nullptr;
     std::vector<HtResampleJob *> d_gen_blocks;
+    std::vector<HtDenseTile *> d_dense_tiles;
+    std::vector<HtTapFast *> d_dense_taps;
+    std::vector<HtResampleJob *> d_pruned_tiles;
+    bool pruned_built = false;
     HtTileRec *d_tile_recs = nullptr;
     HtScanScale *d_scales = nullptr;
     HtResampleJob *d_tail_jobs = nullptr;
@@ -114,6 +118,8 @@
     bool rs_group_forced = false;
     int rs_rpt = 4;
     bool rs_bands = true;
+    bool rs_prune = true;
+    int rs_dense = -1;
 
     uint8_t *d_frames_own = nullptr;
     size_t d_frames_own_bytes = 0;
@@ -320,6 +326,7 @@
 ht_status ht_frames_own_reserve(ht_ctx *ctx, size_t need, const char *fn);
 void ht_frames_bind_own(ht_ctx *ctx, int n);
 ht_status ht_launch_pyramid(ht_ctx *ctx, uint32_t flags);
+ht_status ht_launch_pruned_planes(ht_ctx *ctx, int nframes);
 ht_status ht_launch_scan(ht_ctx *ctx, uint32_t flags);
 ht_status ht_launch_scan_early(ht_ctx *ctx, uint32_t flags);
 bool ht_scan_is_builtin_cascade(const uint8_t *blob, size_t len);
diff --git a/headtrackr_amd/csrc/ht_plan_types.h b/headtrackr_amd/csrc/ht_plan_types.h
--- a/headtrackr_amd/csrc/ht_plan_types.h
+++ b/headtrackr_amd/csrc/ht_plan_types.h
@@ -51,6 +51,25 @@
 };
 constexpr int HT_RSB_ROWS = 24;
 
+struct HtDenseTile {
+    uint32_t src_off, dst_off;
+    int32_t src_stride, dst_stride;
+    int32_t sx, sy, sw, sh;
+    int32_t dw, dh;
+    int32_t cw, ch;
+    double rx, ry;
+    int32_t X0, Y0;
+    uint16_t ncg, R;
+    uint16_t np, mode;
+    uint32_t lane_magic;
+    uint32_t pad;
+    int32_t ex_xa, ex_ya;
+    int32_t ex_sw16, ex_sh;
+    uint32_t band_ya4, band_sh4;
+    uint32_t tap_col, tap_row;
+};
+static_assert(sizeof(HtDenseTile) == 120, "HtDenseTile");
+
 constexpr int HT_SCAN_TXH = 64;
 constexpr int HT_SCAN_TYH = 32;
 struct HtScanScale {
@@ -86,6 +105,8 @@
     bool tail_table_forced;
     bool early_scan, aux_stream;
     uint32_t queue_capacity_cfg;
+    bool rs_dense = false;
+    bool rs_prune = false;
 };
 
 struct HtGeometryPlan {
@@ -93,8 +114,11 @@
     uint64_t arena_stride = 0;
     uint64_t pyr_bytes = 0, windows_per_frame = 0;
     std::vector<std::vector<HtResampleJob>> gens;
+    std::vector<std::vector<HtResampleJob>> pruned_gens, pruned_tiles;
     std::vector<std::vector<HtResampleJob>> gen_tiles;
     std::vector<uint32_t> gen_blocks;
+    std::vector<std::vector<HtDenseTile>> dense_tiles;
+    std::vector<std::vector<HtTapFast>> dense_taps;
     int tail_first_gen = 0;
     int tail_table = 0;
     std::vector<HtResampleJob> tail_jobs;
diff --git a/headtrackr_amd/csrc/ht_pyramid.hip b/headtrackr_amd/csrc/ht_pyramid.hip
--- a/headtrackr_amd/csrc/ht_pyramid.hip
+++ b/headtrackr_amd/csrc/ht_pyramid.hip
@@ -459,27 +459,34 @@
 #define RSB_T(var_)
 #endif
 typedef __attribute__((address_space(3))) void rs_lds_void;
-template <int RPT>
-__global__ __launch_bounds__(256, RSB_WPS) void k_resample_bands(const HtResampleJob *__restrict__ tiles, uint8_t *__restrict__ arena,
+template <int RPT, bool DENSE>
+__global__ __launch_bounds__(256, RSB_WPS) void k_resample_bands(const std::conditional_t<DENSE, HtDenseTile, HtResampleJob> *__restrict__ tiles,
+                                                                    const HtTapFast *__restrict__ taps, uint8_t *__restrict__ arena,
                                                                     uint64_t arena_stride, uint32_t blocks_per_frame, uint32_t ngroups,
                                                                     uint32_t nframes, uint32_t group_frames) {
+    using Rec = std::conditional_t<DENSE, HtDenseTile, HtResampleJob>;
     constexpr int TH = 16 * RPT;
     __shared__ __attribute__((aligned(16))) uint8_t s_src[4 * RSB_BAND];
-    __shared__ RsTap s_col[RS_TW], s_row[TH];
+    __shared__ RsTap s_col[DENSE ? 1 : RS_TW], s_row[DENSE ? 1 : TH];
     uint32_t gidx, blk;
     if (!xcd_item(blocks_per_frame, ngroups, &gidx, &blk)) return;
 #ifdef HT_RS_PHASES
     unsigned long long rsb_t_entry = 0, rsb_t0 = 0, rsb_t1 = 0, rsb_t2 = 0, rsb_t3 = 0, rsb_t4 = 0, rsb_acc[7] = {0, 0, 0, 0, 0, 0, 0};
     RSB_T(rsb_t_entry);
 #endif
-    const HtResampleJob J = tiles[blk];
+    const Rec J = tiles[blk];
     const uint32_t f0 = gidx * group_frames, f1 = min(f0 + group_frames, nframes);
     const int tid = (int)threadIdx.x;
     const int np = (int)J.np;
-    const int X0 = (int)J.bx * RS_TW, Y0 = (int)J.pass0 * 16;
+    int X0, Y0, ncg, R, rstep;
+    uint32_t mode;
+    if constexpr (DENSE) {
+        X0 = J.X0, Y0 = J.Y0, ncg = (int)J.ncg, R = (int)J.R, rstep = R, mode = J.mode;
+    } else {
+        X0 = (int)J.bx * RS_TW, Y0 = (int)J.pass0 * 16, ncg = 16, R = 4, rstep = 4, mode = J.pad;
+    }
     uint8_t *frame = arena + (uint64_t)f0 * arena_stride;
-    const int ncols = min(RS_TW, J.dw - X0), nrows = min(16 * np, J.dh - Y0);
-    const uint32_t mode = J.pad;
+    const int ncols = min(4 * ncg, J.dw - X0), nrows = min(4 * R * np, J.dh - Y0);
     if ((mode & 4u) && ncols > 0 && nrows > 0) {
         const int w = __builtin_amdgcn_readfirstlane(tid >> 6), l = tid & 63;
         const int xa = J.ex_xa, sw16 = J.ex_sw16;
@@ -501,22 +508,38 @@
         _Pragma("unroll") for (int i = 0; i < 4; i++) if (on[i])                                                                         \
             __builtin_amdgcn_raw_ptr_buffer_load_lds(fr_, (rs_lds_void *)(band + i * 1024), 16, voff[i], soff_, 0, 0);                   \
     } while (0)
+        int lr = l >> 4;
+        if constexpr (DENSE) lr = (int)(((uint32_t)l * J.lane_magic) >> 16);
+        const bool lane_live = !DENSE || lr < R;
+        const int lrc = DENSE ? min(lr, R - 1) : lr;
+        const int cbase = (l - lr * ncg) * 4, x0 = X0 + cbase;
+        const int yt = Y0 + R * np * w + lrc;
+        const int npx = min(4, J.dw - x0);
+        uint4 c01, c23;
+        if constexpr (DENSE) {
+            const uint4 *tc = reinterpret_cast<const uint4 *>(taps + J.tap_col + cbase);
+            c01 = tc[0], c23 = tc[1];
+        }
         {
             const __amdgpu_buffer_rsrc_t fr = RS_FRAME_RSRC(fbase);
             RSB_DMA(fr, 0u);
-            if (tid < ncols) s_col[tid] = rs_tap(X0 + tid, J.rx, J.sw, J.sx);
-            if (tid >= 64 && tid - 64 < nrows) s_row[tid - 64] = rs_tap(Y0 + tid - 64, J.ry, J.sh, J.sy);
-        }
-        __syncthreads();
-        const int cbase = (l & 15) * 4, x0 = X0 + cbase;
-        const int yt = Y0 + 4 * np * w + (l >> 4);
-        const int npx = min(4, J.dw - x0);
+            if constexpr (!DENSE) {
+                if (tid < ncols) s_col[tid] = rs_tap(X0 + tid, J.rx, J.sw, J.sx);
+                if (tid >= 64 && tid - 64 < nrows) s_row[tid - 64] = rs_tap(Y0 + tid - 64, J.ry, J.sh, J.sy);
+            }
+        }
+        if constexpr (!DENSE) __syncthreads();
         int ia[4];
         float ctf[4];
-#pragma unroll
-        for (int k = 0; k < 4; k++) {
-            const RsTap *ct = &s_col[min(cbase + k, ncols - 1)];
-            ia[k] = ct->a - xa, ctf[k] = (float)ct->t;
+        if constexpr (DENSE) {
+            ia[0] = (int)c01.x, ia[1] = (int)c01.z, ia[2] = (int)c23.x, ia[3] = (int)c23.z;
+            ctf[0] = __uint_as_float(c01.y), ctf[1] = __uint_as_float(c01.w), ctf[2] = __uint_as_float(c23.y), ctf[3] = __uint_as_float(c23.w);
+        } else {
+#pragma unroll
+            for (int k = 0; k < 4; k++) {
+                const RsTap *ct = &s_col[min(cbase + k, ncols - 1)];
+                ia[k] = ct->a - xa, ctf[k] = (float)ct->t;
+            }
         }
         uint32_t one = 1u;
         asm volatile("" : "+s"(one));
@@ -524,7 +547,6 @@
         const int dh = J.dh, ch = J.ch, dst_stride = J.dst_stride;
         const uint32_t doff = J.dst_off + (uint32_t)(yt * dst_stride + x0);
         const uint32_t pxmask = npx >= 4 ? 0xffffffffu : (npx <= 0 ? 0u : ((1u << (8 * npx)) - 1u));
-        const int ia8 = npx > 0 ? ia[0] : 0;
         auto frames = [&](auto NPc, auto BOXc) {
             constexpr int NP = decltype(NPc)::value;
             constexpr bool BOX = decltype(BOXc)::value;
@@ -533,13 +555,21 @@
             bool st[NP], rv[NP];
 #pragma unroll
             for (int q = 0; q < NP; q++) {
-                const int y = yt + 4 * q;
-                const RsTap *ry = &s_row[min(y - Y0, nrows - 1)];
-                roff[q] = (uint32_t)((ry->a - yaw) * RS_SP + w * RSB_BAND);
-                rtf[q] = (float)ry->t;
+                const int y = yt + rstep * q;
+                if constexpr (DENSE) {
+                    const HtTapFast rt = taps[J.tap_row + (uint32_t)(y - Y0)];
+                    roff[q] = (uint32_t)(rt.a * RS_SP + w * RSB_BAND);
+                    rtf[q] = rt.tf;
+                } else {
+                    const RsTap *ry = &s_row[min(y - Y0, nrows - 1)];
+                    roff[q] = (uint32_t)((ry->a - yaw) * RS_SP + w * RSB_BAND);
+                    rtf[q] = (float)ry->t;
+                }
                 rv[q] = y < dh;
-                st[q] = y < ch && x0 < dst_stride;
-            }
+                st[q] = lane_live && y < ch && x0 < dst_stride;
+            }
+            if constexpr (DENSE) __builtin_amdgcn_s_waitcnt(0x0f70);
+            const int ia8 = npx > 0 ? ia[0] : 0;
             for (uint32_t f = f0; f < f1; f++) {
                 asm volatile("" : "+s"(fbase));
                 const __amdgpu_buffer_rsrc_t fr = RS_FRAME_RSRC(fbase);
@@ -595,14 +625,29 @@
                             uint32_t roff_f = roff[q];
                             int yrel = yt - Y0, cb = cbase;
                             asm volatile("" : "+v"(roff_f), "+v"(yrel), "+v"(cb));
-                            const RsTap *ry = &s_row[min(yrel + 4 * q, nrows - 1)];
                             const uint8_t *rowf = s_src + roff_f;
-#pragma unroll
-                            for (int k = 0; k < 4; k++) {
-                                if (__builtin_fabsf(d[k]) >= thr) {
-                                    const RsTap *ct = &s_col[min(cb + k, ncols - 1)];
-                                    oq &= ~(0xffu << (8 * k));
-                                    oq |= rs_pixel_f64(rowf + ia[k], rowf + ia[k] + one, ct->u, ct->t, ry->u, ry->t) << (8 * k);
+                            if constexpr (DENSE) {
+                                uint32_t blk_f = blk;
+                                asm volatile("" : "+s"(blk_f));
+                                const Rec &Jf = tiles[blk_f];
+                                const RsTap ry = rs_tap(Y0 + min(yrel + rstep * q, nrows - 1), Jf.ry, Jf.sh, Jf.sy);
+#pragma unroll
+                                for (int k = 0; k < 4; k++) {
+                                    if (__builtin_fabsf(d[k]) >= thr) {
+                                        const RsTap ct = rs_tap(X0 + min(cb + k, ncols - 1), Jf.rx, Jf.sw, Jf.sx);
+                                        oq &= ~(0xffu << (8 * k));
+                                        oq |= rs_pixel_f64(rowf + ia[k], rowf + ia[k] + one, ct.u, ct.t, ry.u, ry.t) << (8 * k);
+                                    }
+                                }
+                            } else {
+                                const RsTap *ry = &s_row[min(yrel + 4 * q, nrows - 1)];
+#pragma unroll
+                                for (int k = 0; k < 4; k++) {
+                                    if (__builtin_fabsf(d[k]) >= thr) {
+                                        const RsTap *ct = &s_col[min(cb + k, ncols - 1)];
+                                        oq &= ~(0xffu << (8 * k));
+                                        oq |= rs_pixel_f64(rowf + ia[k], rowf + ia[k] + one, ct->u, ct->t, ry->u, ry->t) << (8 * k);
+                                    }
                                 }
                             }
                         }
@@ -623,7 +668,7 @@
                 }
 #pragma unroll
                 for (int q = 0; q < NP; q++)
-                    if (st[q]) __builtin_amdgcn_raw_buffer_store_b32(o[q], fr, doff, (uint32_t)(4 * q * dst_stride), 0);
+                    if (st[q]) __builtin_amdgcn_raw_buffer_store_b32(o[q], fr, doff, (uint32_t)(rstep * q * dst_stride), 0);
 #ifdef HT_RS_PHASES
                 RSB_T(rsb_t4);
                 if (f + 1 < f1) {
@@ -659,8 +704,16 @@
 #undef RS_FRAME_RSRC
         return;
     }
-    const HtResampleJob &Jm = tiles[blk];
-    const int x0 = X0 + (tid & 15) * 4, yt = Y0 + (tid >> 4);
+    const Rec &Jm = tiles[blk];
+    int x0, yt, ystep;
+    bool lane_live = true;
+    if constexpr (DENSE) {
+        const int l = tid & 63, lr = (int)(((uint32_t)l * Jm.lane_magic) >> 16);
+        lane_live = lr < R;
+        x0 = X0 + (l - lr * ncg) * 4, yt = Y0 + R * np * (tid >> 6) + min(lr, R - 1), ystep = R;
+    } else {
+        x0 = X0 + (tid & 15) * 4, yt = Y0 + (tid >> 4), ystep = 16;
+    }
     const int npx = min(4, Jm.dw - x0);
     const bool drawn = ncols > 0 && nrows > 0;
     RsTap cx[4];
@@ -672,13 +725,13 @@
         asm volatile("" : "+v"(ytl));
 #pragma unroll
         for (int q = 0; q < RPT; q++) {
-            const int y = ytl + 16 * q;
+            const int y = ytl + ystep * q;
             uint32_t o = 0;
             if (drawn && q < np && y < Jm.dh && npx > 0) {
                 const RsTap ry = rs_tap(y, Jm.ry, Jm.sh, Jm.sy);
                 o = rs_pixels4<const uint8_t *>(src + (size_t)ry.a * Jm.src_stride, src + (size_t)ry.b * Jm.src_stride, cx, ry, 0, npx);
             }
-            if (q < np && y < Jm.ch && x0 < Jm.dst_stride) *reinterpret_cast<uint32_t *>(frame + Jm.dst_off + (size_t)y * Jm.dst_stride + x0) = o;
+            if (lane_live && q < np && y < Jm.ch && x0 < Jm.dst_stride) *reinterpret_cast<uint32_t *>(frame + Jm.dst_off + (size_t)y * Jm.dst_stride + x0) = o;
         }
     }
 }
@@ -922,17 +975,22 @@
         char gname[24];
         std::snprintf(gname, sizeof(gname), "resample_g%d", (int)g);
         HtProfScope ps(c, c->rs_gennames ? gname : "resample");
+        const bool dense = c->rs_bands && g < c->plan.dense_tiles.size() && !c->plan.dense_tiles[g].empty();
+        const uint32_t nblocks = dense ? (uint32_t)c->plan.dense_tiles[g].size() : c->plan.gen_blocks[g];
         uint32_t K = 1;
         const uint32_t kmax = (uint32_t)((!c->rs_group_forced && (int64_t)c->W * c->H >= 400000) ? std::min(c->rs_group, 4) : c->rs_group);
-        while (K * 2 <= kmax && (uint64_t)c->plan.gen_blocks[g] * ((uint32_t)c->nframes / (K * 2)) >= (uint64_t)c->rs_min_wgs &&
+        while (K * 2 <= kmax && (uint64_t)nblocks * ((uint32_t)c->nframes / (K * 2)) >= (uint64_t)c->rs_min_wgs &&
                (uint32_t)c->nframes % (K * 2 * 8) == 0)
             K *= 2;
         if (c->dbg_rs_k > 0) K = (uint32_t)std::min(c->dbg_rs_k, std::max(1, c->nframes));
         const uint32_t ngroups = ((uint32_t)c->nframes + K - 1) / K;
-        const dim3 rgrid((c->plan.gen_blocks[g] * ngroups + 7u) & ~7u);
-        if (c->rs_bands)
-            hipLaunchKernelGGL(k_resample_bands<HT_RS_MAX_PASSES>, rgrid, dim3(256), 0, c->stream, c->d_gen_blocks[g], c->d_arena, c->plan.arena_stride,
-                               c->plan.gen_blocks[g], ngroups, (uint32_t)c->nframes, K);
+        const dim3 rgrid((nblocks * ngroups + 7u) & ~7u);
+        if (dense)
+            hipLaunchKernelGGL((k_resample_bands<HT_RS_MAX_PASSES, true>), rgrid, dim3(256), 0, c->stream, c->d_dense_tiles[g], c->d_dense_taps[g], c->d_arena,
+                               c->plan.arena_stride, nblocks, ngroups, (uint32_t)c->nframes, K);
+        else if (c->rs_bands)
+            hipLaunchKernelGGL((k_resample_bands<HT_RS_MAX_PASSES, false>), rgrid, dim3(256), 0, c->stream, c->d_gen_blocks[g], (const HtTapFast *)nullptr, c->d_arena,
+                               c->plan.arena_stride, nblocks, ngroups, (uint32_t)c->nframes, K);
         else
             hipLaunchKernelGGL(k_resample<HT_RS_MAX_PASSES>, rgrid, dim3(256), 0, c->stream, c->d_gen_blocks[g], c->d_arena, c->plan.arena_stride,
                                c->plan.gen_blocks[g], ngroups, (uint32_t)c->nframes, K);
@@ -953,6 +1011,29 @@
         else
             hipLaunchKernelGGL(k_resample_tail_f64, dim3(((uint32_t)c->nframes + 7u) & ~7u), dim3(TAILF_NT), 0, c->stream, c->d_tail_jobs, c->d_tail_prefix,
                                c->plan.tail, c->d_arena, c->plan.arena_stride, (uint32_t)c->nframes);
+        HT_HIP(c, hipGetLastError());
+    }
+    return HT_OK;
+}
+
+ht_status ht_launch_pruned_planes(ht_ctx *c, int nframes) {
+    const HtGeometryPlan &P = c->plan;
+    if (c->d_pruned_tiles.size() != P.pruned_tiles.size()) c->d_pruned_tiles.assign(P.pruned_tiles.size(), nullptr);
+    for (size_t g = 1; g < P.pruned_tiles.size(); g++) {
+        const std::vector<HtResampleJob> &tiles = P.pruned_tiles[g];
+        if (tiles.empty()) continue;
+        if (!c->d_pruned_tiles[g]) {
+            HT_HIP(c, hipMalloc(&c->d_pruned_tiles[g], tiles.size() * sizeof(HtResampleJob)));
+            HT_HIP(c, hipMemcpy(c->d_pruned_tiles[g], tiles.data(), tiles.size() * sizeof(HtResampleJob), hipMemcpyHostToDevice));
+        }
+        const uint32_t nblocks = (uint32_t)tiles.size();
+        const dim3 rgrid((nblocks * (uint32_t)nframes + 7u) & ~7u);
+        if (c->rs_bands)
+            hipLaunchKernelGGL((k_resample_bands<HT_RS_MAX_PASSES, false>), rgrid, dim3(256), 0, c->stream, c->d_pruned_tiles[g], (const HtTapFast *)nullptr, c->d_arena,
+                               P.arena_stride, nblocks, (uint32_t)nframes, (uint32_t)nframes, 1u);
+        else
+            hipLaunchKernelGGL(k_resample<HT_RS_MAX_PASSES>, rgrid, dim3(256), 0, c->stream, c->d_pruned_tiles[g], c->d_arena, P.arena_stride, nblocks,
+                               (uint32_t)nframes, (uint32_t)nframes, 1u);
         HT_HIP(c, hipGetLastError());
     }
     return HT_OK;
```

New measurement: 1.071 million frames/s. 0.919x the previous value.
